# nmndeep/Robust-Segmentation

Hardware: AMD Instinct MI355X
Metric: SEA attack-iterations/sec (UperNet-CNX-T, 512x512) (higher is better)
Workload: dtype f32 (frozen-weight GEMMs on the 16-bit matrix cores by operand splitting: fp16x2 (22 significant bits per operand, 3 MFMA products) forward, fp16x2 (22 significant bits per operand, 3 MFMA products) input gradient; fp32 storage and accumulate)

## Files before the change

include/sea_hip.h:

```cpp
#ifndef SEA_HIP_H
#define SEA_HIP_H

#include <stddef.h>
#include <stdint.h>

#ifdef __cplusplus
extern "C" {
#endif

#define SEA_MODE_MASK_CE 0
#define SEA_MODE_MASK_CE_BAL 1
#define SEA_MODE_JS 2
#define SEA_MODE_CE 3

#define SEA_DTYPE_F32 0
#define SEA_DTYPE_BF16 1
#define SEA_DTYPE_F16 2

#define SEA_LAYOUT_NCHW 0
#define SEA_LAYOUT_NHWC 1

int sea_abi_version(void);
const char* sea_build_info(void);
#define SEA_CONFIG_XCD_ORDER 0
// ... 26 lines not shown
#define SEA_K2_VARIANT_DEFAULT 0u
#define SEA_K2_VEC_MASK 0xfu
#define SEA_K2_TUNE_SHIFT 4
#define SEA_K2_STREAM_SHIFT 8
#define SEA_K2_NO_SPLIT (15u << SEA_K2_STREAM_SHIFT)
#define SEA_K2_REG_ONLY 0x1000u
int sea_loss_fwd_bwd_tuned(const void* logits, int dtype, int layout, const void* y, int y_bytes,
                           const float* w, int mode, int track_mode, int B, int C, int64_t HW,
                           float grad_scale, void* dlogits, void* pred, int pred_bytes, float* loss_px,
                           void* workspace, size_t workspace_bytes, float* loss_sum, float* track_sum,
                           int32_t* n_correct, void* stream, int variant);
int sea_loss_plan(int dtype, int layout, int C, int64_t HW, int want_grad, size_t logits_addr, size_t dlogits_addr,
                  unsigned variant, int32_t out[8]);

size_t sea_loss_upsampled_workspace_bytes(int B, int C, int h, int w, int H, int W, int pow2);
int sea_loss_fwd_bwd_upsampled(const float* low, const void* y, int y_bytes, const float* w, int mode,
                               int track_mode, int B, int C, int h, int wl, int H, int W, float grad_scale,
                               float* dlow, void* pred, int pred_bytes, void* workspace,
                               size_t workspace_bytes, float* loss_sum, float* track_sum,
                               int32_t* n_correct, int pow2, void* stream);

int sea_class_counts(const void* pred, int pred_bytes, const void* y, int y_bytes, int B, int C,
                     int64_t HW, int mask_pred, int per_image, int64_t* inter, int64_t* pred_cnt,
                     int64_t* tgt_cnt, void* stream);
int sea_confusion(const void* pred, int pred_bytes, const void* y, int y_bytes, int64_t n, int C,
                  int64_t* hist, void* stream);

int sea_apgd_track(const float* loss_sum, const float* track_sum, const int32_t* n_correct,
                   const int32_t* n_ignored, int B, int64_t HW, int iter, int n_iter, int check_k,
                   int early_stop, int init, int32_t* acc_cnt, float* acc, float* loss_best,
                   float* loss_best_last, float* reduced_last, float* step, float* loss_steps,
                   uint8_t* flags, int32_t* done, const void* loss_workspace, void* stream);
int sea_apgd_linf_step_graph(const float* x, float* x_adv, float* x_old, const float* grad, const float* step_b,
                             const float* eps_dev, const int32_t* iter_dev, int B, int64_t n_per_img, void* stream);
int sea_apgd_track_graph(const float* loss_sum, const float* track_sum, const int32_t* n_correct,
                         const int32_t* n_ignored, int B, int64_t HW, int32_t* iter_dev, const int32_t* check_table,
                         const int32_t* n_iter_dev, int early_stop, int32_t* acc_cnt, float* acc, float* loss_best,
                         float* loss_best_last, float* reduced_last, float* step, float* loss_steps, uint8_t* flags,
                         int32_t* done, const void* loss_workspace, void* stream);
int sea_select_copy(const uint8_t* flags, float* x_adv, float* grad, float* x_best,
                    float* grad_best, float* x_best_adv, const void* pred, void* pred_best,
                    int pred_bytes, int B, int64_t n_per_img, int64_t HW, void* stream);

int sea_count_ignored(const void* y, int y_bytes, int B, int64_t HW, int32_t* n_ignored,
                      void* stream);

int sea_worst_miou_greedy(const float* ints, const float* unions, int A, int N, int C,
                          uint32_t* mt_state, int n_rounds, double* miou, int32_t* selected,
                          int32_t* rounds_run);

int sea_dwconv7x7(const float* x, const float* w, const float* bias, float* y, int B, int C, int H,
                  int W, int flip, void* stream);
int sea_dwconv7x7_nhwc(const float* x, const float* wt, const float* bias, float* y, int B, int C,
                       int H, int W, int flip, unsigned ab, void* stream);
int sea_dwconv7x7_nhwc_add(const float* x, const float* wt, const float* bias, const float* addend, float* y, int B,
                           int C, int H, int W, int flip, unsigned ab, void* stream);

int sea_upsample_bilinear_fwd(const float* x, float* y, int64_t planes, int h, int w, int H, int W,
                              void* stream);
int sea_upsample_bilinear_bwd(const float* gy, float* gx, int64_t planes, int h, int w, int H, int W,
                              void* stream);
int sea_upsample_bilinear_nhwc_fwd(const float* x, const float* residual, float* y, int B, int C, int h,
                                   int w, int H, int W, int64_t y_pixel_stride, void* stream);
int sea_upsample_bilinear_nhwc_bwd(const float* gy, float* gx, int B, int C, int h, int w, int H, int W,
                                   int64_t gy_pixel_stride, void* stream);
#define SEA_UP_NCHW_FWD 0
#define SEA_UP_NCHW_BWD 1
#define SEA_UP_NHWC_FWD 2
#define SEA_UP_NHWC_BWD 3
#define SEA_UP_TAP_FWD 4
#define SEA_UP_TAP_BWD 5
int sea_upsample_plan(int op, int64_t planes_or_batch, int C, int h, int w, int H, int W, int64_t pixel_stride,
                      size_t src_addr, size_t dst_addr, int general_only, int xcd_order, int32_t out[20]);

int64_t sea_wino_tiles(int B, int H, int W, int m);
int sea_wino_input_transform(const float* x, int64_t x_pixel_stride, const float* gate, const float* scale,
                             float* V, int64_t v_tile_stride, int B, int C, int H, int W, int m, int vec4, void* stream);
int sea_wino_filter_transform(const float* w, float* U, int Cout, int Cin, int m, int flip, void* stream);
int sea_wino_input_transform_amax(const float* x, int64_t x_pixel_stride, const float* gate, const float* scale, float* V,
                                  int64_t v_tile_stride, int B, int C, int H, int W, int m, int vec4, uint32_t* amax_out,
                                  void* stream);
int sea_wino_output_transform(const float* M, const float* addend, const float* scale, const float* bias,
                              int relu, float* y, int B, int C, int H, int W, int m, int vec4, void* stream);

int sea_layernorm_fwd(const float* x, const float* w, const float* b, float* y, float* mean, float* rstd,
                      int64_t rows, int C, float eps, void* stream);
int sea_layernorm_bwd(const float* g, const float* x, const float* w, const float* mean, const float* rstd,
                      float* dx, int64_t rows, int C, void* stream);

int64_t sea_layernorm_bwd_params_workspace(int64_t rows, int C);
int sea_layernorm_bwd_params(const float* g, const float* x, const float* w, const float* mean, const float* rstd,
                             float* dx, float* dw, float* db, float* ws, int64_t rows, int C, void* stream);

int sea_block_tail_fwd(const float* x, const float* y, const float* gamma, const float* s, float* out, int64_t rows, int HW,
                       int C, void* stream);
int64_t sea_block_tail_bwd_workspace(int64_t rows, int C);
int sea_block_tail_bwd(const float* g, const float* y, const float* gamma, const float* s, float* gy, float* ggamma, float* ws,
                       int64_t rows, int HW, int C, void* stream);

int64_t sea_dwconv7x7_nhwc_wgrad_workspace(int B, int C, int H);
int sea_dwconv7x7_nhwc_wgrad(const float* x, const float* gy, float* gw, float* gb, float* ws, int B, int C, int H, int W,
                             void* stream);

int sea_adaptive_avg_pool_nhwc_fwd(const float* x, float* out, int B, int C, int H, int W, int oh, int ow, void* stream);
int sea_adaptive_avg_pool_nhwc_bwd(const float* g, float* dx, int B, int C, int H, int W, int oh, int ow, void* stream);

int sea_stem_conv1_ln_gelu(const float* x, const float* w, const float* bias, const float* gamma, const float* beta,
                           float* y, float* a, int B, int CO, int H, int W, float eps, void* stream);
int sea_stem_conv1_bwd(const float* dy, const float* w, float* dx, int B, int CO, int H, int W, void* stream);
int sea_ln_gelu_cl_fwd(const float* y, const float* gamma, const float* beta, float* a, int a_nchw, int B, int C, int64_t HW,
                       float eps, void* stream);
int sea_ln_gelu_cl_bwd(const float* da, int a_nchw, const float* y, const float* gamma, const float* beta, float* dy, int B,
                       int C, int64_t HW, float eps, void* stream);

int sea_tap_gather_fwd(const float* G, float* extra, int accumulate, int B, int C, int h, int w, int H, int W,
                       int inner, void* stream);
int sea_tap_gather_bwd(const float* gz, float* dG, int B, int C, int h, int w, int H, int W, void* stream);
int sea_gate_scale(const float* g, const float* gate, const float* scale, float* out, int64_t pixels, int C,
                   void* stream);

int sea_nchw_to_nhwc(const float* in, const float* scale, float* out, int B, int C, int64_t HW, void* stream);
int sea_nhwc_to_nchw(const float* in, const float* scale, const float* residual, float* out, int B, int C,
                     int64_t HW, void* stream);

int sea_patch2x2(const float* src, float* dst, int B, int H, int W, int C, int inverse, void* stream);

int sea_attention_bwd_terms(const float* q, const float* k, const float* v, int64_t sb, int64_t sh, int64_t st, int B, int H,
                            int T, int D, float scale, const float* out, const float* grad_out, const float* lse,
                            float* delta, float* dq, float* dk, float* dv, int64_t gsb, int64_t gsh, int64_t gst,
                            int terms, void* stream);
int sea_attention_fwd_terms(const float* q, const float* k, const float* v, int64_t sb, int64_t sh, int64_t st, int B, int H,
                            int T, int D, float scale, float* out, float* lse, int terms, void* stream);
int sea_attention_fwd_f16(const float* q, const float* k, const float* v, int64_t sb, int64_t sh, int64_t st, int B, int H,
                          int T, int D, float scale, uint32_t* amax_ws, float* out, float* lse, void* stream);
int sea_attention_bwd_f16(const float* q, const float* k, const float* v, int64_t sb, int64_t sh, int64_t st, int B, int H,
                          int T, int D, float scale, const float* out, const float* grad_out, const float* lse,
                          float* delta, uint32_t* amax_ws, float* dq, float* dk, float* dv, int64_t gsb, int64_t gsh,
                          int64_t gst, void* stream);

#define SEA_GEMM_VARIANT_DEFAULT 0u
#define SEA_GEMM_PIPE_SINGLE 1u
#define SEA_GEMM_PIPE_PINGPONG 2u
#define SEA_GEMM_PIPE_BIG 3u
#define SEA_GEMM_PIPE_MASK 3u
#define SEA_GEMM_SHAPE16 4u
int sea_gemm_plan(int M, int N, int K, int terms, int batch, int64_t lda, int64_t ldc, int64_t ld_addend, int prologue, int fused,
                  unsigned variant, int32_t out[16]);
int64_t sea_gemm_split_packed_bytes(int N, int K, int terms);
int sea_absmax_bits(const float* A, int64_t lda, int M, int K, int batch, int64_t strideA, int rows_per_word,
                    uint32_t* out_bits, void* stream);
int sea_gemm_split_f16(const float* A, int64_t lda, const void* Wp, float* C, int64_t ldc, const float* bias, int relu, int M,
                       int N, int K, int batch, int64_t strideA, int64_t strideW_bytes, int64_t strideC,
                       const uint32_t* amax_bits, int amax_rows, uint32_t* out_amax, unsigned variant, void* stream);
int sea_gemm_split_pack(const float* W, int64_t ldw, int trans, int N, int K, int terms, void* out, void* stream);
int sea_gemm_splitk_reduce(const float* partial, int splits, int M, int N, const float* bias, const float* addend,
                           int64_t ld_addend, int relu, float* C, int64_t ldc, uint32_t* out_amax, void* stream);
typedef struct SeaGemmEpilogue {
  const float* addend;
  int64_t ld_addend, stride_addend;
  float* gelu_out;
  const float* gelu_grad_of;
  const float* a_gelu_grad_of;
  int a_gate;
  int a_gelu;
  float a_amax_mul;
  const float* a_amax_mul_dev;
} SeaGemmEpilogue;
int sea_gemm_split_fused(const float* A, int64_t lda, const void* Wp, float* C, int64_t ldc, const float* bias, int relu, int M,
                         int N, int K, int terms, int batch, int64_t strideA, int64_t strideW_bytes, int64_t strideC,
                         const uint32_t* amax_bits, int amax_rows, uint32_t* out_amax, const SeaGemmEpilogue* epi,
                         unsigned variant, void* stream);
int sea_gemm_split(const float* A, int64_t lda, const void* Wp, float* C, int64_t ldc, const float* bias, int relu, int M,
                   int N, int K, int terms, int batch, int64_t strideA, int64_t strideW_bytes, int64_t strideC,
                   unsigned variant, void* stream);
int sea_classifier_supported(int P, int K, int cls);
int sea_classifier_fwd(const float* y, const float* W, const float* bias, float* out, int B, int P, int K, int cls, void* stream);
int sea_classifier_bwd(const float* g, const float* W, float* gy, int B, int P, int K, int cls, const float* gate,
                       const float* gate_scale, void* stream);
int sea_mlp_fused_supported(int C, int H);
int sea_ln_mlp_fused_fwd(const float* x, int64_t ldx, const float* ln_w, const float* ln_b, float ln_eps, const void* W1p,
                         const float* b1, const void* W2p, const float* b2, const float* res, int64_t ldres, float* y,
                         int64_t ldy, int M, int C, int H, const uint32_t* amax_x, const uint32_t* amax_h, void* stream);
int sea_ln_mlp_fused_bwd(const float* g, int64_t ldg, const float* x, int64_t ldx, const float* ln_w, const float* ln_b,
                         float ln_eps, const void* W1p, const float* b1, const void* W2tp, const void* W1tp, float* dx,
                         int64_t lddx, int M, int C, int H, const uint32_t* amax_x, const float* amax_mul_dev, void* stream);
int sea_probe_gelu_mismatches(unsigned long long* out, void* stream);
int sea_probe_ln_rows(const float* x, const float* ln_w, const float* ln_b, float eps, int M, int C, float* yn, float* mean,
                      float* rstd, void* stream);
int sea_mlp_fused_stamps(int bwd, const float* g, int64_t ldg, const float* x, int64_t ldx, const void* W1p, const float* b1,
                         const void* W2p, const void* W1tp, const float* b2, const float* res, float* y, int M, int C,
                         const uint32_t* amax_x, const uint32_t* amax_h, const float* amax_mul_dev, unsigned long long* dbg,
                         void* stream);
int sea_mlp_fused_fwd(const float* x, int64_t ldx, const void* W1p, const float* b1, const void* W2p, const float* b2,
                      const float* res, int64_t ldres, float* y, int64_t ldy, int M, int C, int H, const uint32_t* amax_x,
                      const uint32_t* amax_h, void* stream);
int sea_mlp_fused_bwd(const float* g, int64_t ldg, const float* x, int64_t ldx, const void* W1p, const float* b1,
                      const void* W2tp, const void* W1tp, float* dx, int64_t lddx, int M, int C, int H,
                      const uint32_t* amax_x, const float* amax_mul_dev, void* stream);
int sea_probe_stream_copy(const void* src, void* dst, size_t bytes, int non_temporal, void* stream);
int sea_probe_stream_read(const void* src, float* sink, size_t bytes, void* stream);

#define SEA_MSF_MAX_CLASSES 192
int sea_msf_resize_input(const float* x, float* y, float* y_flip, int64_t planes, int h, int w, int H, int W,
                         void* stream);
int sea_msf_accumulate(const float* logits, float* score, int B, int C, int hl, int wl, int Hs, int Ws, int H, int W,
                       int flip, void* stream);

#define SEA_SW_MAX_ANCHORS 32
int sea_sw_merge(const float* logits, float* out, int B, int C, int hl, int wl, int ws, const int* h_anchors, int n_h,
                 const int* w_anchors, int n_w, int H, int W, int flip, int softmax, int accumulate, void* stream);
int sea_sw_finish(const float* avg, float* score, int B, int C, int H, int W, int Ho, int Wo, int flip, int accumulate,
                  void* stream);

int sea_psp_polyphase_split(const float* x, float* y, int B, int H, int W, int C, int d, int first_only, void* stream);
int sea_psp_polyphase_merge(const float* y, float* x, int B, int H, int W, int C, int d, int first_only, void* stream);
int sea_psp_upsample_ac(const float* x, float* y, int64_t planes, int h, int w, int H, int W, void* stream);
int sea_psp_upsample_ac_bwd(const float* gy, float* gx, float* work, int64_t planes, int h, int w, int H, int W,
                            void* stream);
int sea_psp_upsample_ac_nhwc(const float* x, float* y, int B, int C, int h, int w, int H, int W, int S, void* stream);
int sea_psp_upsample_ac_nhwc_bwd(const float* gy, float* gx, float* work, int B, int C, int h, int w, int H, int W,
                                 int S, void* stream);
int sea_psp_add_relu(const float* a, const float* r, float* y, int64_t n, void* stream);
int sea_psp_add_relu_bwd(const float* gy, const float* y, float* gx, int64_t n, void* stream);

int64_t sea_bn_train_workspace_floats(int64_t M, int C);
int sea_bn_train_fwd(const float* x, const float* r, const float* gamma, const float* beta, float* y, float* mean,
                     float* invstd, float* scale, float* running_mean, float* running_var, int64_t* num_batches_tracked,
                     float* work, int64_t M, int C, float eps, float momentum, int relu, void* stream);
int sea_bn_train_bwd(const float* g, const float* x, const float* y, const float* mean, const float* invstd,
                     const float* scale, float* dx, float* dgamma, float* dbeta, float* gr, float* work, int64_t M, int C,
                     int relu, void* stream);

size_t sea_train_ce_workspace_bytes(int B, int64_t HW);
int sea_train_ce_fwd(const void* logits, int dtype, const int64_t* y, const float* w, int64_t ignore_label, float thresh,
                     int reduce_mean, int B, int C, int64_t HW, float* loss_px, void* workspace, size_t workspace_bytes,
                     void* words, void* stream);
int sea_train_ohem_select(float* loss_px, int64_t N, void* workspace, size_t workspace_bytes, void* words, void* stream);
int sea_train_ce_bwd(const void* logits, int dtype, const int64_t* y, const float* w, int64_t ignore_label, int ohem,
                     int B, int C, int64_t HW, const float* loss_px, const float* g, const void* words, void* dlogits,
                     void* stream);

int sea_train_ce_up_tile(int C, int h, int w, int H, int W);
size_t sea_train_ce_up_workspace_bytes(int B, int C, int h, int w, int H, int W);
int sea_train_ce_up_fwd(const float* low, const int64_t* y, const float* wgt, int64_t ignore_label, float thresh,
                        int reduce_mean, int B, int C, int h, int w, int H, int W, float* loss_px, void* workspace,
                        size_t workspace_bytes, void* words, void* stream);
int sea_train_ce_up_bwd(const float* low, const int64_t* y, const float* wgt, int64_t ignore_label, int ohem, int B, int C,
                        int h, int w, int H, int W, const float* loss_px, const float* g, const void* words, float* dlow,
                        void* workspace, size_t workspace_bytes, void* stream);

int sea_train_ce_up_ac_tile(int C, int h, int w, int H, int W);
size_t sea_train_ce_up_ac_workspace_bytes(int B, int C, int h, int w, int H, int W);
int sea_train_ce_up_ac_fwd(const float* low, const int64_t* y, const float* wgt, int64_t ignore_label, float thresh,
                           int reduce_mean, int B, int C, int h, int w, int H, int W, float* loss_px, void* workspace,
                           size_t workspace_bytes, void* words, void* stream);
int sea_train_ce_up_ac_bwd(const float* low, const int64_t* y, const float* wgt, int64_t ignore_label, int ohem, int B,
                           int C, int h, int w, int H, int W, const float* loss_px, const float* g, const void* words,
                           float* dlow, void* workspace, size_t workspace_bytes, void* stream);

int sea_train_ce_up_pow2_supported(int C, int h, int w, int H, int W);
size_t sea_train_ce_up_pow2_workspace_bytes(int B, int C, int h, int w, int H, int W);
// ... 10 lines not shown
```

robust-segmentation_amd/csrc/classifier.hip:

```cpp
#include "sea_common.h"

namespace sea {

typedef float cf32x16 __attribute__((ext_vector_type(16)));
typedef float cf32x4 __attribute__((ext_vector_type(4)));

constexpr int CLS_MAX = 32;

__global__ __launch_bounds__(256, 2) void classifier_fwd_kernel(const float* __restrict__ y, const float* __restrict__ W,
                                                                const float* __restrict__ bias, float* __restrict__ out,
                                                                int tiles, int P, int K, int cls) {
  extern __shared__ __attribute__((aligned(16))) char cls_smem[];
  const int ldw = K + 4;
  float* const Ws = (float*)cls_smem;
  for (int i = threadIdx.x; i < CLS_MAX * (K / 4); i += 256) {
    const int c = i / (K / 4), k4 = i - c * (K / 4);
    const cf32x4 v = c < cls ? *(const cf32x4*)(W + (int64_t)c * K + 4 * k4) : cf32x4{0.f, 0.f, 0.f, 0.f};
    *(cf32x4*)(Ws + c * ldw + 4 * k4) = v;
  }
  __syncthreads();
  const int lane = threadIdx.x & 63, wave = threadIdx.x >> 6;
  const int r = lane & 31, h = lane >> 5;
  const float* const wrow = Ws + r * ldw + 4 * h;
  const int tiles_per_img = P / 32;
  for (int t = blockIdx.x * 4 + wave; t < tiles; t += gridDim.x * 4) {
    const float* const yrow = y + ((int64_t)t * 32 + r) * K + 4 * h;
    cf32x16 acc;
#pragma unroll
    for (int e = 0; e < 16; ++e) acc[e] = 0.f;
    cf32x4 cur[8], nxt[8];
#pragma unroll
    for (int i = 0; i < 8; ++i) cur[i] = *(const cf32x4*)(yrow + 8 * i);
    for (int kk = 0; kk < K; kk += 64) {
      if (kk + 64 < K) {
#pragma unroll
        for (int i = 0; i < 8; ++i) nxt[i] = *(const cf32x4*)(yrow + kk + 64 + 8 * i);
      }
#pragma unroll
      for (int i = 0; i < 8; ++i) {
        const cf32x4 a = *(const cf32x4*)(wrow + kk + 8 * i);
#pragma unroll
        for (int e = 0; e < 4; ++e) acc = __builtin_amdgcn_mfma_f32_32x32x2f32(a[e], cur[i][e], acc, 0, 0, 0);
      }
#pragma unroll
      for (int i = 0; i < 8; ++i) cur[i] = nxt[i];
    }
    const int b = t / tiles_per_img, p0 = (t - b * tiles_per_img) * 32;
    float* const ob = out + (int64_t)b * cls * P + p0 + r;
#pragma unroll
    for (int e = 0; e < 16; ++e) {
      const int c = (e & 3) + 8 * (e >> 2) + 4 * h;
      if (c < cls) ob[(int64_t)c * P] = acc[e] + (bias ? bias[c] : 0.f);
    }
  }
}

template <bool GATE>
__global__ __launch_bounds__(256, 2) void classifier_bwd_kernel(const float* __restrict__ g, const float* __restrict__ W,
                                                                float* __restrict__ gy, int tiles, int P, int K, int cls,
                                                                const float* __restrict__ gate, const float* __restrict__ scale) {
  extern __shared__ __attribute__((aligned(16))) char cls_smem[];
  const int ldw = K + 32;
  const int pairs = (cls + 1) / 2;
  float* const Ws = (float*)cls_smem;
  for (int i = threadIdx.x; i < 2 * pairs * (K / 4); i += 256) {
    const int c = i / (K / 4), k4 = i - c * (K / 4);
    const cf32x4 v = c < cls ? *(const cf32x4*)(W + (int64_t)c * K + 4 * k4) : cf32x4{0.f, 0.f, 0.f, 0.f};
    *(cf32x4*)(Ws + c * ldw + 4 * k4) = v;
  }
  __syncthreads();
  const int lane = threadIdx.x & 63, wave = threadIdx.x >> 6;
  const int r = lane & 31, h = lane >> 5;
  const int tiles_per_img = P / 32;
  for (int t = blockIdx.x * 4 + wave; t < tiles; t += gridDim.x * 4) {
    const int b = t / tiles_per_img, p0 = (t - b * tiles_per_img) * 32;
    const float* const gb = g + (int64_t)b * cls * P + p0 + r;
    float a[CLS_MAX / 2];
#pragma unroll
    for (int s = 0; s < CLS_MAX / 2; ++s) {
      const int c = 2 * s + h;
      a[s] = (s < pairs && c < cls) ? gb[(int64_t)c * P] : 0.f;
    }
    float* const orow = gy + ((int64_t)t * 32 + 4 * h) * K + r;
    const float* const grow = GATE ? gate + ((int64_t)t * 32 + 4 * h) * K + r : nullptr;
    for (int n0 = 0; n0 < K; n0 += 128) {
      cf32x16 acc[4];
      float gt[GATE ? 4 : 1][GATE ? 16 : 1];
      float sc[4];
#pragma unroll
      for (int nt = 0; nt < 4; ++nt) {
#pragma unroll
        for (int e = 0; e < 16; ++e) acc[nt][e] = 0.f;
        if constexpr (GATE) {
          if (n0 + 32 * nt < K) {
            sc[nt] = scale[n0 + 32 * nt + r];
#pragma unroll
            for (int e = 0; e < 16; ++e) gt[nt][e] = grow[(int64_t)((e & 3) + 8 * (e >> 2)) * K + n0 + 32 * nt];
          }
        }
      }
#pragma unroll
      for (int s = 0; s < CLS_MAX / 2; ++s) {
        if (s < pairs) {
          const float* const wr = Ws + (2 * s + h) * ldw + n0 + r;
#pragma unroll
          for (int nt = 0; nt < 4; ++nt)
            if (n0 + 32 * nt < K) acc[nt] = __builtin_amdgcn_mfma_f32_32x32x2f32(a[s], wr[32 * nt], acc[nt], 0, 0, 0);
        }
      }
#pragma unroll
      for (int nt = 0; nt < 4; ++nt) {
        if (n0 + 32 * nt < K) {
#pragma unroll
          for (int e = 0; e < 16; ++e) {
            const int64_t o = (int64_t)((e & 3) + 8 * (e >> 2)) * K + n0 + 32 * nt;
            if constexpr (GATE)
              orow[o] = gt[nt][e] > 0.f ? acc[nt][e] * sc[nt] : 0.f;
            else
              orow[o] = acc[nt][e];
          }
        }
      }
    }
  }
}

}

using namespace sea;

extern "C" int sea_classifier_supported(int P, int K, int cls) {
  return (P > 0 && (P % 32) == 0 && K >= 64 && (K % 64) == 0 && K <= 1024 && cls >= 1 && cls <= CLS_MAX) ? 1 : 0;
}

static int classifier_grid(int tiles) {
  const int blocks = (tiles + 3) / 4;
  return blocks < 512 ? blocks : 512;
}

extern "C" int sea_classifier_fwd(const float* y, const float* W, const float* bias, float* out, int B, int P, int K, int cls,
                                  void* stream) {
  SEA_CHECK_ARG(y && W && out && B > 0 && sea_classifier_supported(P, K, cls));
  SEA_CHECK_ARG(((((uintptr_t)y) | ((uintptr_t)W)) & 15) == 0 && (int64_t)B * P / 32 < (1ll << 30));
  const int tiles = (int)((int64_t)B * P / 32);
  const int lds = CLS_MAX * (K + 4) * 4;
  static bool attr_set_dev[64] = {};
  int dev = 0;
  (void)hipGetDevice(&dev);
  if (!attr_set_dev[dev & 63]) {
    (void)hipFuncSetAttribute((const void*)classifier_fwd_kernel, hipFuncAttributeMaxDynamicSharedMemorySize, CLS_MAX * (1024 + 4) * 4);
    attr_set_dev[dev & 63] = true;
  }
  hipLaunchKernelGGL(classifier_fwd_kernel, dim3(classifier_grid(tiles)), dim3(256), (size_t)lds, (hipStream_t)stream, y, W, bias, out,
                     tiles, P, K, cls);
  SEA_RETURN_LAST();
}

extern "C" int sea_classifier_bwd(const float* g, const float* W, float* gy, int B, int P, int K, int cls, const float* gate,
                                  const float* gate_scale, void* stream) {
  SEA_CHECK_ARG(g && W && gy && B > 0 && sea_classifier_supported(P, K, cls) && ((gate == nullptr) == (gate_scale == nullptr)));
  SEA_CHECK_ARG((((uintptr_t)W) & 15) == 0 && (int64_t)B * P / 32 < (1ll << 30));
  const int tiles = (int)((int64_t)B * P / 32);
  const int lds = 2 * ((cls + 1) / 2) * (K + 32) * 4;
  static bool attr_set_dev[64] = {};
  int dev = 0;
  (void)hipGetDevice(&dev);
  if (!attr_set_dev[dev & 63]) {
    (void)hipFuncSetAttribute((const void*)classifier_bwd_kernel<false>, hipFuncAttributeMaxDynamicSharedMemorySize, CLS_MAX * (1024 + 32) * 4);
    (void)hipFuncSetAttribute((const void*)classifier_bwd_kernel<true>, hipFuncAttributeMaxDynamicSharedMemorySize, CLS_MAX * (1024 + 32) * 4);
    attr_set_dev[dev & 63] = true;
  }
  if (gate)
    hipLaunchKernelGGL(classifier_bwd_kernel<true>, dim3(classifier_grid(tiles)), dim3(256), (size_t)lds, (hipStream_t)stream, g, W, gy,
                       tiles, P, K, cls, gate, gate_scale);
  else
    hipLaunchKernelGGL(classifier_bwd_kernel<false>, dim3(classifier_grid(tiles)), dim3(256), (size_t)lds, (hipStream_t)stream, g, W, gy,
                       tiles, P, K, cls, gate, gate_scale);
  SEA_RETURN_LAST();
}
```

robust-segmentation_amd/csrc/fpn_fused.hip:

```cpp
#include "sea_common.h"
#include <utility>
#include "bilinear_map.h"
#include "upsample_plan.h"

namespace sea {

constexpr int kTB = kTapBlock;

typedef float tg_f4 __attribute__((ext_vector_type(4)));

template <int N, typename F, int... I>
__device__ __forceinline__ void tg_static_for_impl(F&& f, std::integer_sequence<int, I...>) {
  (f(std::integral_constant<int, I>{}), ...);
}
template <int N, typename F>
__device__ __forceinline__ void tg_static_for(F&& f) {
  tg_static_for_impl<N>(f, std::make_integer_sequence<int, N>{});
}

template <int S>
struct TgAxis {
  static constexpr int LOG = Pow2<S>::LOG;
  static constexpr int base(int u0) { return (u0 >> LOG) - 1; }
  static constexpr int k(int u0, int q) { return ((u0 + q) >> LOG) - (u0 >> LOG); }
// ... 200 lines not shown
__global__ __launch_bounds__(256) void tap_gather_bwd_pow2_kernel(const float4* __restrict__ gz, float4* __restrict__ dG,
                                                                  int CG, int h, int w, int64_t total, int xcd,
                                                                  Divs3 dv) {
  constexpr int T = 2 * S, TW = T + 2;
  const int H = h * S, W = w * S;
  const IndexRange rg = xcd_range(total, xcd);
  const bool fast = total < kFastIndexLimit;
  for (int64_t i = rg.begin; i < rg.end; i += rg.stride) {
    const Index4 ix = split_index(i, dv, fast);
    const int cg = ix.c0, xq = ix.c1, yq = ix.c2;
    const int b = (int)ix.c3;
    const bool eL = xq == 0, eR = xq == w - 1, eT = yq == 0, eB = yq == h - 1;
    const int Q0 = S * xq - S / 2 - 1, R0 = S * yq - S / 2 - 1;
    float wxe[T];
#pragma unroll
    for (int t = 0; t < T; ++t) wxe[t] = pow2_tap_weight<S>(t, eL, eR);
    const float4* gb = gz + ((int64_t)b * H * W + Q0) * CG + cg;
    float4 acc[3][3];
#pragma unroll
    for (int a = 0; a < 3; ++a)
#pragma unroll
      for (int bq = 0; bq < 3; ++bq) acc[a][bq] = make_float4(0.f, 0.f, 0.f, 0.f);
#pragma unroll 1
    for (int u = 0; u < TW; ++u) {
      const int R = R0 + u;
      if (R < 0 || R >= H) continue;
      const float wy0 = pow2_tap_weight<S>(u - 2, eT, eB), wy1 = pow2_tap_weight<S>(u - 1, eT, eB),
                  wy2 = pow2_tap_weight<S>(u, eT, eB);
      const float4* row = gb + (int64_t)R * W * CG;
      float4 g[TW];
#pragma unroll
      for (int v = 0; v < TW; ++v) {
        const int Q = Q0 + v;
        g[v] = make_float4(0.f, 0.f, 0.f, 0.f);
        if (Q >= 0 && Q < W) g[v] = row[(int64_t)v * CG];
      }
      float4 rb[3];
#pragma unroll
      for (int bq = 0; bq < 3; ++bq) {
        rb[bq] = make_float4(0.f, 0.f, 0.f, 0.f);
#pragma unroll
        for (int t = 0; t < T; ++t) {
          const int v = t + 2 - bq;
          rb[bq].x = fmaf(wxe[t], g[v].x, rb[bq].x);
          rb[bq].y = fmaf(wxe[t], g[v].y, rb[bq].y);
          rb[bq].z = fmaf(wxe[t], g[v].z, rb[bq].z);
          rb[bq].w = fmaf(wxe[t], g[v].w, rb[bq].w);
        }
      }
#pragma unroll
      for (int bq = 0; bq < 3; ++bq) {
        acc[0][bq].x = fmaf(wy0, rb[bq].x, acc[0][bq].x);
        acc[0][bq].y = fmaf(wy0, rb[bq].y, acc[0][bq].y);
        acc[0][bq].z = fmaf(wy0, rb[bq].z, acc[0][bq].z);
        acc[0][bq].w = fmaf(wy0, rb[bq].w, acc[0][bq].w);
        acc[1][bq].x = fmaf(wy1, rb[bq].x, acc[1][bq].x);
        acc[1][bq].y = fmaf(wy1, rb[bq].y, acc[1][bq].y);
        acc[1][bq].z = fmaf(wy1, rb[bq].z, acc[1][bq].z);
        acc[1][bq].w = fmaf(wy1, rb[bq].w, acc[1][bq].w);
        acc[2][bq].x = fmaf(wy2, rb[bq].x, acc[2][bq].x);
        acc[2][bq].y = fmaf(wy2, rb[bq].y, acc[2][bq].y);
        acc[2][bq].z = fmaf(wy2, rb[bq].z, acc[2][bq].z);
        acc[2][bq].w = fmaf(wy2, rb[bq].w, acc[2][bq].w);
      }
    }
    float4* out = dG + (((int64_t)b * h + yq) * w + xq) * 9 * CG + cg;
#pragma unroll
    for (int a = 0; a < 3; ++a)
#pragma unroll
      for (int bq = 0; bq < 3; ++bq) out[(a * 3 + bq) * CG] = acc[a][bq];
  }
}

__global__ __launch_bounds__(256) void gate_scale_kernel(const float4* __restrict__ g, const float4* __restrict__ gate,
                                                         const float4* __restrict__ scale, float4* __restrict__ out, int CG,
                                                         int64_t total) {
  for (int64_t i = (int64_t)blockIdx.x * blockDim.x + threadIdx.x; i < total; i += (int64_t)gridDim.x * blockDim.x) {
    const float4 s = scale[i % CG], gv = g[i], t = gate[i];
    out[i] = make_float4(t.x > 0.f ? gv.x * s.x : 0.f, t.y > 0.f ? gv.y * s.y : 0.f, t.z > 0.f ? gv.z * s.z : 0.f,
                         t.w > 0.f ? gv.w * s.w : 0.f);
  }
}

}

using namespace sea;

extern "C" int sea_tap_gather_fwd(const float* G, float* extra, int accumulate, int B, int C, int h, int w, int H, int W,
                                  int inner, void* stream) {
  SEA_CHECK_ARG(G && extra);
  UpsamplePlan pl;
  SEA_CHECK_ARG(upsample_plan(UpsampleQuery{SEA_UP_TAP_FWD, B, C, h, w, H, W, 0, (uintptr_t)G, (uintptr_t)extra,
                                            process_config().upsample_general != 0, process_config().xcd_order}, &pl) == 0);
  dispatch_s<0, 4, 8>(pl.S, [&](auto S) {
    launch_planned(tap_gather_fwd_kernel<decltype(S)::value>, pl, 1, stream, (const float4*)G, (float4*)extra, accumulate, C / 4,
                   h, w, H, W, (float)h / (float)H, (float)w / (float)W, pl.nbh, pl.nbw, pl.total, pl.xo,
                   divs3(C / 4, pl.nbw, pl.nbh), inner ? 1 : 0);
  });
  SEA_RETURN_LAST();
}

extern "C" int sea_tap_gather_bwd(const float* gz, float* dG, int B, int C, int h, int w, int H, int W, void* stream) {
  SEA_CHECK_ARG(gz && dG);
  UpsamplePlan pl;
  SEA_CHECK_ARG(upsample_plan(UpsampleQuery{SEA_UP_TAP_BWD, B, C, h, w, H, W, 0, (uintptr_t)gz, (uintptr_t)dG,
                                            process_config().upsample_general != 0, process_config().xcd_order}, &pl) == 0);
  if (pl.kernel == UPK_TAP_BWD_POW2)
    dispatch_s<4, 8>(pl.S, [&](auto S) {
      launch_planned(tap_gather_bwd_pow2_kernel<decltype(S)::value>, pl, 1, stream, (const float4*)gz, (float4*)dG, C / 4, h, w,
                     pl.total, pl.xo, divs3(C / 4, w, h));
    });
  else
    launch_planned(tap_gather_bwd_kernel, pl, 1, stream, (const float4*)gz, (float4*)dG, C / 4, h, w, H, W, (float)h / (float)H,
                   (float)w / (float)W, pl.total, pl.xo, divs3(C / 4, w, h));
  SEA_RETURN_LAST();
}

extern "C" int sea_gate_scale(const float* g, const float* gate, const float* scale, float* out, int64_t pixels, int C,
                              void* stream) {
  SEA_CHECK_ARG(g && gate && scale && out && pixels > 0 && C > 0 && (C % 4) == 0);
  SEA_CHECK_ARG(((((uintptr_t)g) | ((uintptr_t)gate) | ((uintptr_t)scale) | ((uintptr_t)out)) & 15) == 0);
  const int64_t total = pixels * (C / 4);
  hipLaunchKernelGGL(gate_scale_kernel, dim3(grid_for(total, 256 * 2)), dim3(256), 0, (hipStream_t)stream,
                     (const float4*)g, (const float4*)gate, (const float4*)scale, (float4*)out, C / 4, total);
  SEA_RETURN_LAST();
}
```

robust-segmentation_amd/csrc/wino_kernels.hip:

```cpp
#include "sea_common.h"

namespace sea {

__host__ __device__ constexpr float wino_bt(int m, int i, int k) {
  if (m == 2) {
    constexpr float T[4][4] = {{1, 0, -1, 0}, {0, 1, 1, 0}, {0, -1, 1, 0}, {0, 1, 0, -1}};
    return T[i][k];
  }
  constexpr float T[6][6] = {{4, 0, -5, 0, 1, 0},  {0, -4, -4, 1, 1, 0}, {0, 4, -4, -1, 1, 0},
                             {0, -2, -1, 2, 1, 0}, {0, 2, -1, -2, 1, 0}, {0, 4, 0, -5, 0, 1}};
  return T[i][k];
}
__host__ __device__ constexpr float wino_g(int m, int i, int k) {
  if (m == 2) {
    constexpr float T[4][3] = {{1, 0, 0}, {0.5f, 0.5f, 0.5f}, {0.5f, -0.5f, 0.5f}, {0, 0, 1}};
    return T[i][k];
  }
  constexpr float T[6][3] = {{1.f / 4, 0, 0},           {-1.f / 6, -1.f / 6, -1.f / 6}, {-1.f / 6, 1.f / 6, -1.f / 6},
                             {1.f / 24, 1.f / 12, 1.f / 6}, {1.f / 24, -1.f / 12, 1.f / 6},  {0, 0, 1}};
  return T[i][k];
}
__host__ __device__ constexpr float wino_at(int m, int i, int k) {
  if (m == 2) {
    constexpr float T[2][4] = {{1, 1, 1, 0}, {0, 1, -1, -1}};
    return T[i][k];
  }
  constexpr float T[4][6] = {{1, 1, 1, 1, 1, 0}, {0, 1, -1, 2, -2, 0}, {0, 1, 1, 4, 4, 0}, {0, 1, -1, 8, -8, 1}};
  return T[i][k];
}

template <int VEC>
__device__ __forceinline__ void axpy(float c, const float (&v)[VEC], float (&acc)[VEC], bool& first) {
  if (c == 0.f) return;
#pragma unroll
  for (int e = 0; e < VEC; ++e) acc[e] = first ? c * v[e] : fmaf(c, v[e], acc[e]);
  first = false;
}

template <int VEC>
struct VecT;
template <>
struct VecT<4> {
  using type = float4;
};
template <>
struct VecT<2> {
  using type = float2;
};

template <int VEC>
__device__ __forceinline__ void vload(const float* p, float (&v)[VEC]) {
  const typename VecT<VEC>::type r = *(const typename VecT<VEC>::type*)p;
  const float* rp = (const float*)&r;
#pragma unroll
  for (int e = 0; e < VEC; ++e) v[e] = rp[e];
}
template <int VEC>
__device__ __forceinline__ void vstore(float* p, const float (&v)[VEC]) {
  typename VecT<VEC>::type r;
  float* rp = (float*)&r;
#pragma unroll
  for (int e = 0; e < VEC; ++e) rp[e] = v[e];
  *(typename VecT<VEC>::type*)p = r;
}

template <int M, int VEC>
__global__ __launch_bounds__(256) void wino_input_kernel(const float* __restrict__ x, const float* __restrict__ gate,
                                                         const float* __restrict__ scale, float* __restrict__ V, int C,
                                                         int H, int W, int nTh, int nTw, int64_t T, int64_t total,
                                                         int64_t xps, int64_t vts, int xcd, Divs3 dv,
                                                         uint32_t* __restrict__ amax_out) {
  constexpr int A = M + 2;
  const bool fast = total < kFastIndexLimit;
  const IndexRange rg = xcd_range(total, xcd);
  for (int64_t idx = rg.begin; idx < rg.end; idx += rg.stride) {
    const Index4 ix = split_index(idx, dv, fast);
    const int cg = ix.c0, tx = ix.c1, ty = ix.c2;
    const int b = (int)ix.c3;
    const int64_t t = ((int64_t)b * nTh + ty) * nTw + tx;
    const int y0 = ty * M - 1, x0 = tx * M - 1;
    const int64_t base = (int64_t)b * H * W * C + (int64_t)cg * VEC;
    const float* xb = x + (int64_t)b * H * W * xps + (int64_t)cg * VEC;
    float sc[VEC];
#pragma unroll
    for (int e = 0; e < VEC; ++e) sc[e] = scale ? scale[cg * VEC + e] : 1.f;
    float d[A][A][VEC];
#pragma unroll
    for (int i = 0; i < A; ++i) {
      const int yy = y0 + i;
#pragma unroll
      for (int j = 0; j < A; ++j) {
        const int xx = x0 + j;
        if (yy >= 0 && yy < H && xx >= 0 && xx < W) {
          vload<VEC>(xb + ((int64_t)yy * W + xx) * xps, d[i][j]);
          if (gate) {
            float gt[VEC];
            vload<VEC>(gate + base + ((int64_t)yy * W + xx) * C, gt);
#pragma unroll
            for (int e = 0; e < VEC; ++e) d[i][j][e] = gt[e] > 0.f ? d[i][j][e] * sc[e] : 0.f;
          }
        } else {
#pragma unroll
          for (int e = 0; e < VEC; ++e) d[i][j][e] = 0.f;
        }
      }
    }
    float tmp[A][A][VEC];
#pragma unroll
    for (int i = 0; i < A; ++i)
#pragma unroll
      for (int j = 0; j < A; ++j) {
        bool first = true;
#pragma unroll
        for (int k = 0; k < A; ++k) axpy<VEC>(wino_bt(M, i, k), d[k][j], tmp[i][j], first);
      }
    float* vb = V + t * vts + (int64_t)cg * VEC;
    uint32_t vmax = 0;
#pragma unroll
    for (int i = 0; i < A; ++i)
#pragma unroll
      for (int j = 0; j < A; ++j) {
        float v[VEC];
        bool first = true;
#pragma unroll
        for (int k = 0; k < A; ++k) axpy<VEC>(wino_bt(M, j, k), tmp[i][k], v, first);
        vstore<VEC>(vb + (int64_t)(i * A + j) * T * vts, v);
#pragma unroll
        for (int e = 0; e < VEC; ++e) {
          const uint32_t b = __float_as_uint(v[e]) & 0x7fffffffu;
          vmax = b > vmax ? b : vmax;
        }
      }
    if (amax_out != nullptr) {
      const int ti = (int)t;
      const bool whole = __ballot(1) == ~0ull && __all(ti == __shfl(ti, 0, 64));
      if (whole) {
#pragma unroll
        for (int o = 32; o > 0; o >>= 1) {
          const uint32_t other = (uint32_t)__shfl_xor((int)vmax, o, 64);
          vmax = other > vmax ? other : vmax;
        }
        if ((threadIdx.x & 63) == 0) atomicMax(amax_out + t, vmax);
      } else {
        atomicMax(amax_out + t, vmax);
      }
    }
  }
}

template <int M, int VEC>
__global__ __launch_bounds__(256) void wino_input_cols_kernel(const float* __restrict__ x, const float* __restrict__ gate,
                                                              const float* __restrict__ scale, float* __restrict__ V, int C,
                                                              int H, int W, int nTh, int nTw, int64_t T, int64_t total,
                                                              int64_t xps, int64_t vts, int xcd, Divs3 dv,
                                                              uint32_t* __restrict__ amax_out) {
  constexpr int A = M + 2;
  const bool fast = total < kFastIndexLimit;
  const IndexRange rg = xcd_range(total, xcd);
  for (int64_t idx = rg.begin; idx < rg.end; idx += rg.stride) {
    const Index4 ix = split_index(idx, dv, fast);
    const int cg = ix.c0, tx = ix.c1, ty = ix.c2;
    const int b = (int)ix.c3;
    const int64_t t = ((int64_t)b * nTh + ty) * nTw + tx;
    const int y0 = ty * M - 1, x0 = tx * M - 1;
    const int64_t base = (int64_t)b * H * W * C + (int64_t)cg * VEC;
    const float* xb = x + (int64_t)b * H * W * xps + (int64_t)cg * VEC;
    float sc[VEC];
#pragma unroll
    for (int e = 0; e < VEC; ++e) sc[e] = scale ? scale[cg * VEC + e] : 1.f;
    float tmp[A][A][VEC];
#pragma unroll
    for (int j = 0; j < A; ++j) {
      const int xx = x0 + j;
      float col[A][VEC];
#pragma unroll
      for (int i = 0; i < A; ++i) {
        const int yy = y0 + i;
        if (yy >= 0 && yy < H && xx >= 0 && xx < W) {
          vload<VEC>(xb + ((int64_t)yy * W + xx) * xps, col[i]);
          if (gate) {
            float gt[VEC];
            vload<VEC>(gate + base + ((int64_t)yy * W + xx) * C, gt);
#pragma unroll
            for (int e = 0; e < VEC; ++e) col[i][e] = gt[e] > 0.f ? col[i][e] * sc[e] : 0.f;
          }
        } else {
#pragma unroll
          for (int e = 0; e < VEC; ++e) col[i][e] = 0.f;
        }
      }
#pragma unroll
      for (int i = 0; i < A; ++i) {
        bool first = true;
#pragma unroll
        for (int k = 0; k < A; ++k) axpy<VEC>(wino_bt(M, i, k), col[k], tmp[i][j], first);
      }
    }
    float* vb = V + t * vts + (int64_t)cg * VEC;
    uint32_t vmax = 0;
#pragma unroll
    for (int i = 0; i < A; ++i)
#pragma unroll
      for (int j = 0; j < A; ++j) {
        float v[VEC];
        bool first = true;
#pragma unroll
        for (int k = 0; k < A; ++k) axpy<VEC>(wino_bt(M, j, k), tmp[i][k], v, first);
        vstore<VEC>(vb + (int64_t)(i * A + j) * T * vts, v);
#pragma unroll
        for (int e = 0; e < VEC; ++e) {
          const uint32_t b = __float_as_uint(v[e]) & 0x7fffffffu;
          vmax = b > vmax ? b : vmax;
        }
      }
    if (amax_out != nullptr) {
      const int ti = (int)t;
      const bool whole = __ballot(1) == ~0ull && __all(ti == __shfl(ti, 0, 64));
      if (whole) {
#pragma unroll
        for (int o = 32; o > 0; o >>= 1) {
          const uint32_t other = (uint32_t)__shfl_xor((int)vmax, o, 64);
          vmax = other > vmax ? other : vmax;
        }
        if ((threadIdx.x & 63) == 0) atomicMax(amax_out + t, vmax);
      } else {
        atomicMax(amax_out + t, vmax);
      }
    }
  }
}

template <int M, int VEC>
__global__ __launch_bounds__(256) void wino_output_kernel(const float* __restrict__ Mx, const float* __restrict__ addend,
                                                          const float* __restrict__ scale,
                                                          const float* __restrict__ bias, int relu,
                                                          float* __restrict__ y, int C, int H, int W, int nTh, int nTw,
                                                          int64_t T, int64_t total, Divs3 dv) {
  constexpr int A = M + 2;
  const bool fast = total < kFastIndexLimit;
  for (int64_t idx = (int64_t)blockIdx.x * blockDim.x + threadIdx.x; idx < total;
       idx += (int64_t)gridDim.x * blockDim.x) {
    const Index4 ix = split_index(idx, dv, fast);
    const int cg = ix.c0, tx = ix.c1, ty = ix.c2;
    const int b = (int)ix.c3;
    const int64_t t = ((int64_t)b * nTh + ty) * nTw + tx;
    const float* mb = Mx + t * C + (int64_t)cg * VEC;
    float tmp[M][A][VEC];
#pragma unroll
    for (int j = 0; j < A; ++j) {
      float col[A][VEC];
#pragma unroll
      for (int i = 0; i < A; ++i) vload<VEC>(mb + (int64_t)(i * A + j) * T * C, col[i]);
#pragma unroll
      for (int p = 0; p < M; ++p) {
        bool first = true;
#pragma unroll
        for (int i = 0; i < A; ++i) axpy<VEC>(wino_at(M, p, i), col[i], tmp[p][j], first);
      }
    }
    float bv[VEC], sv[VEC];
#pragma unroll
    for (int e = 0; e < VEC; ++e) {
      bv[e] = bias ? bias[cg * VEC + e] : 0.f;
      sv[e] = scale ? scale[cg * VEC + e] : 1.f;
    }
    float* yb = y + (int64_t)b * H * W * C + (int64_t)cg * VEC;
#pragma unroll
    for (int p = 0; p < M; ++p) {
      const int yy = ty * M + p;
#pragma unroll
      for (int q = 0; q < M; ++q) {
        const int xx = tx * M + q;
        float o[VEC];
        bool first = true;
#pragma unroll
        for (int j = 0; j < A; ++j) axpy<VEC>(wino_at(M, q, j), tmp[p][j], o, first);
        if (addend && yy < H && xx < W) {
          float ad[VEC];
          vload<VEC>(addend + (int64_t)b * H * W * C + ((int64_t)yy * W + xx) * C + (int64_t)cg * VEC, ad);
#pragma unroll
          for (int e = 0; e < VEC; ++e) o[e] += ad[e];
        }
#pragma unroll
        for (int e = 0; e < VEC; ++e) {
          o[e] = scale ? fmaf(o[e], sv[e], bv[e]) : o[e] + bv[e];
          if (relu) o[e] = fmaxf(o[e], 0.f);
        }
        if (yy < H && xx < W) vstore<VEC>(yb + ((int64_t)yy * W + xx) * C, o);
      }
    }
  }
}

template <int M>
__global__ __launch_bounds__(256) void wino_filter_kernel(const float* __restrict__ w, float* __restrict__ U, int Cout,
                                                          int Cin, int flip) {
  constexpr int A = M + 2;
  const int64_t n = (int64_t)Cout * Cin;
  for (int64_t idx = (int64_t)blockIdx.x * blockDim.x + threadIdx.x; idx < n; idx += (int64_t)gridDim.x * blockDim.x) {
    const int c = (int)(idx % Cin);
    const int o = (int)(idx / Cin);
    float g[3][3];
#pragma unroll
    for (int a = 0; a < 3; ++a)
#pragma unroll
      for (int bq = 0; bq < 3; ++bq) g[a][bq] = w[idx * 9 + (flip ? (2 - a) * 3 + (2 - bq) : a * 3 + bq)];
    float tmp[A][3];
#pragma unroll
    for (int i = 0; i < A; ++i)
#pragma unroll
      for (int j = 0; j < 3; ++j) {
        float s = 0.f;
#pragma unroll
        for (int k = 0; k < 3; ++k)
          if (wino_g(M, i, k) != 0.f) s = fmaf(wino_g(M, i, k), g[k][j], s);
        tmp[i][j] = s;
      }
    const int64_t off = flip ? (int64_t)o * Cin + c : (int64_t)c * Cout + o;
#pragma unroll
    for (int i = 0; i < A; ++i)
#pragma unroll
      for (int j = 0; j < A; ++j) {
        float s = 0.f;
#pragma unroll
        for (int k = 0; k < 3; ++k)
          if (wino_g(M, j, k) != 0.f) s = fmaf(wino_g(M, j, k), tmp[i][k], s);
        U[(int64_t)(i * A + j) * n + off] = s;
      }
  }
}

}

using namespace sea;

static bool wino_dims(int B, int C, int H, int W, int m, int vec, int* nTh, int* nTw, int64_t* T) {
  if (!(B > 0 && C > 0 && H > 0 && W > 0 && (m == 2 || m == 4) && (C % vec) == 0)) return false;
  *nTh = (H + m - 1) / m;
  *nTw = (W + m - 1) / m;
  *T = (int64_t)B * *nTh * *nTw;
  return true;
}

extern "C" int64_t sea_wino_tiles(int B, int H, int W, int m) {
  if (!(B > 0 && H > 0 && W > 0 && (m == 2 || m == 4))) return 0;
  return (int64_t)B * ((H + m - 1) / m) * ((W + m - 1) / m);
}

static int wino_input_impl(const float* x, int64_t x_pixel_stride, const float* gate, const float* scale, float* V,
                           int64_t v_tile_stride, int B, int C, int H, int W, int m, int vec4, uint32_t* amax_out, void* stream);

extern "C" int sea_wino_input_transform(const float* x, int64_t x_pixel_stride, const float* gate, const float* scale,
                                        float* V, int64_t v_tile_stride, int B, int C, int H, int W, int m, int vec4,
                                        void* stream) {
  return wino_input_impl(x, x_pixel_stride, gate, scale, V, v_tile_stride, B, C, H, W, m, vec4, nullptr, stream);
}

extern "C" int sea_wino_input_transform_amax(const float* x, int64_t x_pixel_stride, const float* gate, const float* scale,
                                             float* V, int64_t v_tile_stride, int B, int C, int H, int W, int m, int vec4,
                                             uint32_t* amax_out, void* stream) {
  SEA_CHECK_ARG(amax_out != nullptr);
  return wino_input_impl(x, x_pixel_stride, gate, scale, V, v_tile_stride, B, C, H, W, m, vec4, amax_out, stream);
}

static int wino_input_impl(const float* x, int64_t x_pixel_stride, const float* gate, const float* scale, float* V,
                           int64_t v_tile_stride, int B, int C, int H, int W, int m, int vec4, uint32_t* amax_out, void* stream) {
  int nTh, nTw;
  int64_t T;
  SEA_CHECK_ARG(x && V && wino_dims(B, C, H, W, m, 4, &nTh, &nTw, &T));
  SEA_CHECK_ARG(x_pixel_stride >= C && (x_pixel_stride % 4) == 0);
  SEA_CHECK_ARG(v_tile_stride >= C && (v_tile_stride % 4) == 0);
  SEA_CHECK_ARG(((((uintptr_t)x) | ((uintptr_t)V) | ((uintptr_t)gate)) & 15) == 0);
  if (m == 2) {
    const int64_t total = T * (C / 4);
    hipLaunchKernelGGL((wino_input_kernel<2, 4>), dim3(grid_for_xcd(total, 256)), dim3(256), 0, (hipStream_t)stream, x, gate,
                       scale, V, C, H, W, nTh, nTw, T, total, x_pixel_stride, v_tile_stride, xcd_order_enabled() == 2, divs3(C / 4, nTw, nTh),
                       amax_out);
  } else if (vec4) {
    const int64_t total = T * (C / 4);
    hipLaunchKernelGGL((wino_input_cols_kernel<4, 4>), dim3(grid_for_xcd(total, 256)), dim3(256), 0, (hipStream_t)stream, x, gate,
                       scale, V, C, H, W, nTh, nTw, T, total, x_pixel_stride, v_tile_stride, xcd_order_enabled() == 2, divs3(C / 4, nTw, nTh),
                       amax_out);
  } else {
    const int64_t total = T * (C / 2);
    hipLaunchKernelGGL((wino_input_kernel<4, 2>), dim3(grid_for_xcd(total, 256)), dim3(256), 0, (hipStream_t)stream, x, gate,
                       scale, V, C, H, W, nTh, nTw, T, total, x_pixel_stride, v_tile_stride, xcd_order_enabled() == 2, divs3(C / 2, nTw, nTh),
                       amax_out);
  }
  SEA_RETURN_LAST();
}

extern "C" int sea_wino_output_transform(const float* Mx, const float* addend, const float* scale, const float* bias,
                                         int relu, float* y, int B, int C, int H, int W, int m, int vec4, void* stream) {
  int nTh, nTw;
  int64_t T;
  SEA_CHECK_ARG(Mx && y && wino_dims(B, C, H, W, m, 4, &nTh, &nTw, &T));
  SEA_CHECK_ARG(((((uintptr_t)Mx) | ((uintptr_t)y) | ((uintptr_t)addend)) & 15) == 0);
  if (m == 2) {
    const int64_t total = T * (C / 4);
    hipLaunchKernelGGL((wino_output_kernel<2, 4>), dim3(grid_for(total, 256)), dim3(256), 0, (hipStream_t)stream, Mx,
                       addend, scale, bias, relu, y, C, H, W, nTh, nTw, T, total, divs3(C / 4, nTw, nTh));
  } else if (vec4) {
    const int64_t total = T * (C / 4);
    hipLaunchKernelGGL((wino_output_kernel<4, 4>), dim3(grid_for(total, 256)), dim3(256), 0, (hipStream_t)stream, Mx,
                       addend, scale, bias, relu, y, C, H, W, nTh, nTw, T, total, divs3(C / 4, nTw, nTh));
  } else {
    const int64_t total = T * (C / 2);
    hipLaunchKernelGGL((wino_output_kernel<4, 2>), dim3(grid_for(total, 256)), dim3(256), 0, (hipStream_t)stream, Mx,
                       addend, scale, bias, relu, y, C, H, W, nTh, nTw, T, total, divs3(C / 2, nTw, nTh));
  }
  SEA_RETURN_LAST();
}

extern "C" int sea_wino_filter_transform(const float* w, float* U, int Cout, int Cin, int m, int flip, void* stream) {
  SEA_CHECK_ARG(w && U && Cout > 0 && Cin > 0 && (m == 2 || m == 4));
  const int64_t n = (int64_t)Cout * Cin;
  if (m == 2)
    hipLaunchKernelGGL((wino_filter_kernel<2>), dim3(grid_for(n, 256)), dim3(256), 0, (hipStream_t)stream, w, U, Cout,
                       Cin, flip);
  else
    hipLaunchKernelGGL((wino_filter_kernel<4>), dim3(grid_for(n, 256)), dim3(256), 0, (hipStream_t)stream, w, U, Cout,
                       Cin, flip);
  SEA_RETURN_LAST();
}
```

robust-segmentation_amd/semseg/_native.py:

```python
from __future__ import annotations

import ctypes as C
import os
from typing import Optional

import torch

_PKG = os.path.dirname(os.path.dirname(os.path.abspath(__file__)))
LIB_PATH = os.environ.get("SEA_HIP_LIB", os.path.join(_PKG, "lib", "libsea_hip.so"))

MODE_BY_NAME = {"mask-ce-avg": 0, "mask-ce-bal": 1, "js-avg": 2, "ce": 3, "ce-avg": 3}
DTYPE_CODE = {torch.float32: 0, torch.bfloat16: 1, torch.float16: 2}
LAYOUT_NCHW, LAYOUT_NHWC = 0, 1

_lib = None

_vp, _i, _i64, _f, _sz, _u = C.c_void_p, C.c_int, C.c_int64, C.c_float, C.c_size_t, C.c_uint
_SIGS = {
    "sea_abi_version": (C.c_int, []),
    "sea_build_info": (C.c_char_p, []),
    "sea_fastdiv_magic": (_i, [C.c_uint32, C.POINTER(C.c_uint32), C.POINTER(C.c_uint32)]),
    "sea_apgd_linf_step": (_i, [_vp, _vp, _vp, _vp, _vp, _f, _f, _vp, _i, _i64, _vp]),
    "sea_apgd_l2_workspace_bytes": (_i64, [_i]),
    "sea_apgd_l2_step": (_i, [_vp, _vp, _vp, _vp, _vp, _f, _f, _vp, _vp, _i, _i64, _vp]),
    "sea_linf_random_start": (_i, [_vp, _vp, _f, _vp, _i64, _vp]),
    "sea_linf_project": (_i, [_vp, _vp, _f, _vp, _i64, _vp]),
    "sea_pgd_linf_step": (_i, [_vp, _vp, _vp, _f, _f, _vp, _vp, _i, _i64, _vp]),
    "sea_loss_workspace_bytes": (_sz, [_i, _i64]),
    "sea_loss_fwd_bwd": (_i, [_vp, _i, _i, _vp, _i, _vp, _i, _i, _i, _i, _i64, _f, _vp, _vp, _i, _vp, _vp, _sz,
                              _vp, _vp, _vp, _vp]),
    "sea_loss_fwd_bwd_tuned": (_i, [_vp, _i, _i, _vp, _i, _vp, _i, _i, _i, _i, _i64, _f, _vp, _vp, _i, _vp, _vp,
                                    _sz, _vp, _vp, _vp, _vp, _i]),
    "sea_loss_plan": (_i, [_i, _i, _i, _i64, _i, _sz, _sz, _u, C.POINTER(C.c_int32)]),
    "sea_loss_upsampled_workspace_bytes": (_sz, [_i, _i, _i, _i, _i, _i, _i]),
    "sea_loss_fwd_bwd_upsampled": (_i, [_vp, _vp, _i, _vp, _i, _i, _i, _i, _i, _i, _i, _i, _f, _vp, _vp, _i, _vp, _sz, _vp,
                                        _vp, _vp, _i, _vp]),
    "sea_class_counts": (_i, [_vp, _i, _vp, _i, _i, _i, _i64, _i, _i, _vp, _vp, _vp, _vp]),
    "sea_confusion": (_i, [_vp, _i, _vp, _i, _i64, _i, _vp, _vp]),
    "sea_apgd_track": (_i, [_vp, _vp, _vp, _vp, _i, _i64, _i, _i, _i, _i, _i, _vp, _vp, _vp, _vp, _vp, _vp, _vp,
                            _vp, _vp, _vp, _vp]),
    "sea_apgd_linf_step_graph": (_i, [_vp, _vp, _vp, _vp, _vp, _vp, _vp, _i, _i64, _vp]),
    "sea_apgd_track_graph": (_i, [_vp, _vp, _vp, _vp, _i, _i64, _vp, _vp, _vp, _i, _vp, _vp, _vp, _vp, _vp, _vp, _vp, _vp,
                                  _vp, _vp, _vp]),
    "sea_select_copy": (_i, [_vp, _vp, _vp, _vp, _vp, _vp, _vp, _vp, _i, _i, _i64, _i64, _vp]),
    "sea_count_ignored": (_i, [_vp, _i, _i, _i64, _vp, _vp]),
    "sea_worst_miou_greedy": (_i, [_vp, _vp, _i, _i, _i, _vp, _i, _vp, _vp, _vp]),
    "sea_dwconv7x7": (_i, [_vp, _vp, _vp, _vp, _i, _i, _i, _i, _i, _vp]),
    "sea_dwconv7x7_nhwc": (_i, [_vp, _vp, _vp, _vp, _i, _i, _i, _i, _i, _u, _vp]),
    "sea_dwconv7x7_nhwc_add": (_i, [_vp, _vp, _vp, _vp, _vp, _i, _i, _i, _i, _i, _u, _vp]),
    "sea_nchw_to_nhwc": (_i, [_vp, _vp, _vp, _i, _i, _i64, _vp]),
    "sea_nhwc_to_nchw": (_i, [_vp, _vp, _vp, _vp, _i, _i, _i64, _vp]),
    "sea_upsample_bilinear_fwd": (_i, [_vp, _vp, _i64, _i, _i, _i, _i, _vp]),
    "sea_upsample_bilinear_bwd": (_i, [_vp, _vp, _i64, _i, _i, _i, _i, _vp]),
    "sea_layernorm_fwd": (_i, [_vp, _vp, _vp, _vp, _vp, _vp, _i64, _i, _f, _vp]),
    "sea_layernorm_bwd": (_i, [_vp, _vp, _vp, _vp, _vp, _vp, _i64, _i, _vp]),
    "sea_layernorm_bwd_params_workspace": (_i64, [_i64, _i]),
    "sea_layernorm_bwd_params": (_i, [_vp, _vp, _vp, _vp, _vp, _vp, _vp, _vp, _vp, _i64, _i, _vp]),
    "sea_block_tail_fwd": (_i, [_vp, _vp, _vp, _vp, _vp, _i64, _i, _i, _vp]),
    "sea_block_tail_bwd_workspace": (_i64, [_i64, _i]),
    "sea_block_tail_bwd": (_i, [_vp, _vp, _vp, _vp, _vp, _vp, _vp, _i64, _i, _i, _vp]),
    "sea_dwconv7x7_nhwc_wgrad_workspace": (_i64, [_i, _i, _i]),
    "sea_dwconv7x7_nhwc_wgrad": (_i, [_vp, _vp, _vp, _vp, _vp, _i, _i, _i, _i, _vp]),
    "sea_adaptive_avg_pool_nhwc_fwd": (_i, [_vp, _vp, _i, _i, _i, _i, _i, _i, _vp]),
    "sea_adaptive_avg_pool_nhwc_bwd": (_i, [_vp, _vp, _i, _i, _i, _i, _i, _i, _vp]),
    "sea_stem_conv1_ln_gelu": (_i, [_vp, _vp, _vp, _vp, _vp, _vp, _vp, _i, _i, _i, _i, _f, _vp]),
    "sea_stem_conv1_bwd": (_i, [_vp, _vp, _vp, _i, _i, _i, _i, _vp]),
    "sea_ln_gelu_cl_fwd": (_i, [_vp, _vp, _vp, _vp, _i, _i, _i, _i64, _f, _vp]),
    "sea_ln_gelu_cl_bwd": (_i, [_vp, _i, _vp, _vp, _vp, _vp, _i, _i, _i64, _f, _vp]),
    "sea_wino_tiles": (_i64, [_i, _i, _i, _i]),
    "sea_wino_input_transform": (_i, [_vp, _i64, _vp, _vp, _vp, _i64, _i, _i, _i, _i, _i, _i, _vp]),
    "sea_wino_filter_transform": (_i, [_vp, _vp, _i, _i, _i, _i, _vp]),
    "sea_wino_output_transform": (_i, [_vp, _vp, _vp, _vp, _i, _vp, _i, _i, _i, _i, _i, _i, _vp]),
    "sea_tap_gather_fwd": (_i, [_vp, _vp, _i, _i, _i, _i, _i, _i, _i, _i, _vp]),
    "sea_tap_gather_bwd": (_i, [_vp, _vp, _i, _i, _i, _i, _i, _i, _vp]),
    "sea_gate_scale": (_i, [_vp, _vp, _vp, _vp, _i64, _i, _vp]),
    "sea_upsample_bilinear_nhwc_fwd": (_i, [_vp, _vp, _vp, _i, _i, _i, _i, _i, _i, _i64, _vp]),
    "sea_upsample_bilinear_nhwc_bwd": (_i, [_vp, _vp, _i, _i, _i, _i, _i, _i, _i64, _vp]),
    "sea_upsample_plan": (_i, [_i, _i64, _i, _i, _i, _i, _i, _i64, _sz, _sz, _i, _i, C.POINTER(C.c_int32)]),
    "sea_patch2x2": (_i, [_vp, _vp, _i, _i, _i, _i, _i, _vp]),
    "sea_attention_bwd_terms": (_i, [_vp, _vp, _vp, _i64, _i64, _i64, _i, _i, _i, _i, _f, _vp, _vp, _vp, _vp, _vp, _vp, _vp,
                                     _i64, _i64, _i64, _i, _vp]),
    "sea_attention_fwd_terms": (_i, [_vp, _vp, _vp, _i64, _i64, _i64, _i, _i, _i, _i, _f, _vp, _vp, _i, _vp]),
    "sea_attention_fwd_f16": (_i, [_vp, _vp, _vp, _i64, _i64, _i64, _i, _i, _i, _i, _f, _vp, _vp, _vp, _vp]),
    "sea_attention_bwd_f16": (_i, [_vp, _vp, _vp, _i64, _i64, _i64, _i, _i, _i, _i, _f, _vp, _vp, _vp, _vp, _vp, _vp, _vp, _vp,
                                   _i64, _i64, _i64, _vp]),
    "sea_absmax_bits": (_i, [_vp, _i64, _i, _i, _i, _i64, _i, _vp, _vp]),
    "sea_gemm_split_f16": (_i, [_vp, _i64, _vp, _vp, _i64, _vp, _i, _i, _i, _i, _i, _i64, _i64, _i64, _vp, _i, _vp, _u, _vp]),
    "sea_wino_input_transform_amax": (_i, [_vp, _i64, _vp, _vp, _vp, _i64, _i, _i, _i, _i, _i, _i, _vp, _vp]),
    "sea_gemm_split_fused": (_i, [_vp, _i64, _vp, _vp, _i64, _vp, _i, _i, _i, _i, _i, _i, _i64, _i64, _i64, _vp, _i, _vp, _vp, _u, _vp]),
    "sea_gemm_splitk_reduce": (_i, [_vp, _i, _i, _i, _vp, _vp, _i64, _i, _vp, _i64, _vp, _vp]),
    "sea_gemm_split_packed_bytes": (_i64, [_i, _i, _i]),
    "sea_gemm_split_pack": (_i, [_vp, _i64, _i, _i, _i, _i, _vp, _vp]),
    "sea_gemm_split": (_i, [_vp, _i64, _vp, _vp, _i64, _vp, _i, _i, _i, _i, _i, _i, _i64, _i64, _i64, _u, _vp]),
    "sea_gemm_plan": (_i, [_i, _i, _i, _i, _i, _i64, _i64, _i64, _i, _i, _u, C.POINTER(C.c_int32)]),
    "sea_mlp_fused_supported": (_i, [_i, _i]),
    "sea_classifier_supported": (_i, [_i, _i, _i]),
    "sea_classifier_fwd": (_i, [_vp, _vp, _vp, _vp, _i, _i, _i, _i, _vp]),
    "sea_classifier_bwd": (_i, [_vp, _vp, _vp, _i, _i, _i, _i, _vp, _vp, _vp]),
    "sea_probe_gelu_mismatches": (_i, [_vp, _vp]),
    "sea_probe_ln_rows": (_i, [_vp, _vp, _vp, _f, _i, _i, _vp, _vp, _vp, _vp]),
    "sea_mlp_fused_stamps": (_i, [_i, _vp, _i64, _vp, _i64, _vp, _vp, _vp, _vp, _vp, _vp, _vp, _i, _i, _vp, _vp, _vp, _vp, _vp]),
    "sea_mlp_fused_fwd": (_i, [_vp, _i64, _vp, _vp, _vp, _vp, _vp, _i64, _vp, _i64, _i, _i, _i, _vp, _vp, _vp]),
    "sea_mlp_fused_bwd": (_i, [_vp, _i64, _vp, _i64, _vp, _vp, _vp, _vp, _vp, _i64, _i, _i, _i, _vp, _vp, _vp]),
    "sea_ln_mlp_fused_fwd": (_i, [_vp, _i64, _vp, _vp, _f, _vp, _vp, _vp, _vp, _vp, _i64, _vp, _i64, _i, _i, _i, _vp, _vp, _vp]),
    "sea_ln_mlp_fused_bwd": (_i, [_vp, _i64, _vp, _i64, _vp, _vp, _f, _vp, _vp, _vp, _vp, _vp, _i64, _i, _i, _i, _vp, _vp, _vp]),
    "sea_process_config": (_i, [_i]),
    "sea_probe_stream_copy": (_i, [_vp, _vp, _sz, _i, _vp]),
    "sea_probe_stream_read": (_i, [_vp, _vp, _sz, _vp]),
    "sea_msf_resize_input": (_i, [_vp, _vp, _vp, _i64, _i, _i, _i, _i, _vp]),
    "sea_msf_accumulate": (_i, [_vp, _vp, _i, _i, _i, _i, _i, _i, _i, _i, _i, _vp]),
    "sea_psp_polyphase_split": (_i, [_vp, _vp, _i, _i, _i, _i, _i, _i, _vp]),
    "sea_psp_polyphase_merge": (_i, [_vp, _vp, _i, _i, _i, _i, _i, _i, _vp]),
    "sea_psp_upsample_ac": (_i, [_vp, _vp, _i64, _i, _i, _i, _i, _vp]),
    "sea_psp_upsample_ac_bwd": (_i, [_vp, _vp, _vp, _i64, _i, _i, _i, _i, _vp]),
    "sea_psp_upsample_ac_nhwc": (_i, [_vp, _vp, _i, _i, _i, _i, _i, _i, _i, _vp]),
    "sea_psp_upsample_ac_nhwc_bwd": (_i, [_vp, _vp, _vp, _i, _i, _i, _i, _i, _i, _i, _vp]),
    "sea_psp_add_relu": (_i, [_vp, _vp, _vp, _i64, _vp]),
    "sea_psp_add_relu_bwd": (_i, [_vp, _vp, _vp, _i64, _vp]),
    "sea_bn_train_workspace_floats": (_i64, [_i64, _i]),
    "sea_bn_train_fwd": (_i, [_vp, _vp, _vp, _vp, _vp, _vp, _vp, _vp, _vp, _vp, _vp, _vp, _i64, _i, _f, _f, _i, _vp]),
    "sea_bn_train_bwd": (_i, [_vp, _vp, _vp, _vp, _vp, _vp, _vp, _vp, _vp, _vp, _vp, _i64, _i, _i, _vp]),
    "sea_train_ce_workspace_bytes": (_sz, [_i, _i64]),
    "sea_train_ce_fwd": (_i, [_vp, _i, _vp, _vp, _i64, _f, _i, _i, _i, _i64, _vp, _vp, _sz, _vp, _vp]),
    "sea_train_ohem_select": (_i, [_vp, _i64, _vp, _sz, _vp, _vp]),
    "sea_train_ce_bwd": (_i, [_vp, _i, _vp, _vp, _i64, _i, _i, _i, _i64, _vp, _vp, _vp, _vp, _vp]),
    "sea_train_ce_up_tile": (_i, [_i, _i, _i, _i, _i]),
    "sea_train_ce_up_workspace_bytes": (_sz, [_i, _i, _i, _i, _i, _i]),
    "sea_train_ce_up_fwd": (_i, [_vp, _vp, _vp, _i64, _f, _i, _i, _i, _i, _i, _i, _i, _vp, _vp, _sz, _vp, _vp]),
    "sea_train_ce_up_bwd": (_i, [_vp, _vp, _vp, _i64, _i, _i, _i, _i, _i, _i, _i, _vp, _vp, _vp, _vp, _vp, _sz, _vp]),
    "sea_train_ce_up_ac_tile": (_i, [_i, _i, _i, _i, _i]),
    "sea_train_ce_up_ac_workspace_bytes": (_sz, [_i, _i, _i, _i, _i, _i]),
    "sea_train_ce_up_ac_fwd": (_i, [_vp, _vp, _vp, _i64, _f, _i, _i, _i, _i, _i, _i, _i, _vp, _vp, _sz, _vp, _vp]),
    "sea_train_ce_up_ac_bwd": (_i, [_vp, _vp, _vp, _i64, _i, _i, _i, _i, _i, _i, _i, _vp, _vp, _vp, _vp, _vp, _sz, _vp]),
    "sea_train_ce_up_pow2_supported": (_i, [_i, _i, _i, _i, _i]),
    "sea_train_ce_up_pow2_workspace_bytes": (_sz, [_i, _i, _i, _i, _i, _i]),
    "sea_train_ce_up_pow2_fwd": (_i, [_vp, _vp, _vp, _i64, _i, _i, _i, _i, _i, _i, _vp, _vp, _sz, _vp, _vp]),
    "sea_train_ce_up_pow2_scale": (_i, [_vp, _vp, _vp, _vp, _i64, _vp]),
    "sea_sw_merge": (_i, [_vp, _vp, _i, _i, _i, _i, _i, C.POINTER(C.c_int), _i, C.POINTER(C.c_int), _i, _i, _i, _i, _i, _i,
                          _vp]),
    "sea_sw_finish": (_i, [_vp, _vp, _i, _i, _i, _i, _i, _i, _i, _i, _vp]),
}
EXPORTS = tuple(_SIGS)


class SeaNativeError(RuntimeError):
    pass


def lib():
    global _lib
    if _lib is None:
        if not os.path.exists(LIB_PATH):
            raise SeaNativeError(
                f"libsea_hip.so not found at {LIB_PATH}: build it with "
                "`python robust-segmentation_amd/build_native.py` (there is no CPU fallback)")
        h = C.CDLL(LIB_PATH)
        for name, (res, args) in _SIGS.items():
            fn = getattr(h, name)
            fn.restype, fn.argtypes = res, args
        _lib = h
    return _lib


def _check(rc: int, what: str):
    if rc != 0:
        raise SeaNativeError(f"{what} failed with hipError {rc}")


def _dev(*ts):
    cur = None
    for t in ts:
        if t is None:
            continue
        if not t.is_cuda:
            raise SeaNativeError("libsea_hip works on HIP device tensors only (no CPU fallback); got a CPU tensor")
        if cur is None:
            cur = torch.cuda.current_device()
        if t.device.index != cur:
            raise SeaNativeError(f"tensor on {t.device} but the current device is cuda:{cur}: call "
                                 "torch.cuda.set_device (or use `with torch.cuda.device(...)`) before the launch")

# ... 728 lines not shown

def upsample_bilinear_cl(x, size, out=None, residual=None):
    _dev(x, out, residual)
    if x.dtype != torch.float32 or cl_pixel_stride(x) != x.shape[1]:
        raise SeaNativeError("expected a dense channels_last float32 tensor with C % 4 == 0")
    B, Cc, h, w = x.shape
    H, W = int(size[0]), int(size[1])
    if out is None:
        out = torch.empty(B, Cc, H, W, dtype=torch.float32, device=x.device, memory_format=torch.channels_last)
    S = cl_pixel_stride(out)
    if tuple(out.shape) != (B, Cc, H, W) or S is None:
        raise SeaNativeError("out must be a (B,C,H,W) channels_last tensor or a channel slice of one")
    if residual is not None and (tuple(residual.shape) != (B, Cc, H, W) or cl_pixel_stride(residual) != Cc):
        raise SeaNativeError("residual must be a dense channels_last (B,C,H,W) float32 tensor")
    _check(lib().sea_upsample_bilinear_nhwc_fwd(_p(x), _p(residual), _p(out), B, Cc, h, w, H, W, S, _stream()),
           "sea_upsample_bilinear_nhwc_fwd")
    return out


def upsample_bilinear_backward_cl(gy, in_size):
    _dev(gy)
    S = cl_pixel_stride(gy)
    if S is None:
        raise SeaNativeError("expected a channels_last float32 tensor (or channel slice) with C % 4 == 0")
    B, Cc, H, W = gy.shape
    h, w = int(in_size[0]), int(in_size[1])
    gx = torch.empty(B, Cc, h, w, dtype=torch.float32, device=gy.device, memory_format=torch.channels_last)
    _check(lib().sea_upsample_bilinear_nhwc_bwd(_p(gy), _p(gx), B, Cc, h, w, H, W, S, _stream()),
           "sea_upsample_bilinear_nhwc_bwd")
    return gx


UPSAMPLE_OPS = ("nchw_fwd", "nchw_bwd", "nhwc_fwd", "nhwc_bwd", "tap_fwd", "tap_bwd")
UPSAMPLE_KERNELS = ("nchw_fwd_general", "nchw_fwd_pow2", "nchw_fwd_cells", "nchw_bwd_general", "nchw_bwd_rows", "nchw_bwd_pow2",
                    "nhwc_fwd", "nhwc_fwd_cells", "nhwc_bwd_general", "nhwc_bwd_small", "nhwc_bwd_pow2",
                    "tap_fwd", "tap_bwd_general", "tap_bwd_pow2")
_UPSAMPLE_PLAN_FIELDS = ("kernel", "S", "grid_x", "grid_y", "threads", "lds", "chunk", "nchunks", "total_lo", "total_hi", "xo", "nt",
                         "lcols", "RP", "bands", "per_xcd", "TI", "RMAX", "nbh", "nbw")


def upsample_plan(op: str, n: int, h: int, w: int, H: int, W: int, C_: int = 0, pixel_stride=None, src_addr: int = 0,
                  dst_addr: int = 0, general_only=None, xcd_order=None) -> dict:
    out = (C.c_int32 * len(_UPSAMPLE_PLAN_FIELDS))()
    L = lib()
    general_only = L.sea_process_config(1) if general_only is None else int(bool(general_only))
    xcd_order = L.sea_process_config(0) if xcd_order is None else int(xcd_order)
    rc = L.sea_upsample_plan(UPSAMPLE_OPS.index(op), n, C_, h, w, H, W, C_ if pixel_stride is None else pixel_stride, src_addr,
                             dst_addr, general_only, xcd_order, out)
    plan = dict(zip(_UPSAMPLE_PLAN_FIELDS, out), rc=rc)
    total = (plan.pop("total_hi") << 32) | (plan.pop("total_lo") & 0xffffffff)
    return dict(plan, kernel=UPSAMPLE_KERNELS[plan["kernel"]], total=total)


TAP_INNER = os.environ.get("SEA_TAP_INNER", "1")[:1] != "0"


def tap_gather(G, size, extra=None):
    _dev(G, extra)
    B, h, w, nine, Cc = G.shape
    H, W = int(size[0]), int(size[1])
    if nine != 9:
        raise SeaNativeError("tap_gather: G must be (B,h,w,9,C)")
    acc = extra is not None
    if extra is None:
        extra = torch.empty(B, Cc, H, W, dtype=torch.float32, device=G.device, memory_format=torch.channels_last)
    elif tuple(extra.shape) != (B, Cc, H, W) or cl_pixel_stride(extra) != Cc:
        raise SeaNativeError("tap_gather: extra must be a dense channels_last (B,C,H,W) float32 tensor")
    _check(lib().sea_tap_gather_fwd(_p(_f32c(G)), _p(extra), int(acc), B, Cc, h, w, H, W, int(TAP_INNER), _stream()),
           "sea_tap_gather_fwd")
    return extra


def tap_gather_backward(gz, coarse_size):
    _dev(gz)
    B, Cc, H, W = gz.shape
    if cl_pixel_stride(gz) != Cc:
        raise SeaNativeError("tap_gather_backward: dense channels_last float32 gradient expected")
    h, w = int(coarse_size[0]), int(coarse_size[1])
    dG = torch.empty(B, h, w, 9, Cc, dtype=torch.float32, device=gz.device)
    _check(lib().sea_tap_gather_bwd(_p(gz), _p(dG), B, Cc, h, w, H, W, _stream()), "sea_tap_gather_bwd")
    return dG


def gate_scale(g, gate, scale):
    _dev(g, gate, scale)
    B, Cc, H, W = g.shape
    if cl_pixel_stride(g) != Cc or cl_pixel_stride(gate) != Cc or gate.shape != g.shape or scale.numel() != Cc:
        raise SeaNativeError("gate_scale: dense channels_last float32 tensors of one shape expected")
    out = torch.empty_like(g)
    _check(lib().sea_gate_scale(_p(g), _p(gate), _p(_f32c(scale)), _p(out), B * H * W, Cc, _stream()), "sea_gate_scale")
    return out


def layernorm(x, weight, bias, eps: float):
    _dev(x, weight, bias)
    x = _f32c(x)
    Cc = x.shape[-1]
    rows = x.numel() // Cc
    y = torch.empty_like(x)
    mean = torch.empty(rows, dtype=torch.float32, device=x.device)
    rstd = torch.empty(rows, dtype=torch.float32, device=x.device)
    _check(lib().sea_layernorm_fwd(_p(x), _p(_f32c(weight)), _p(_f32c(bias)), _p(y), _p(mean), _p(rstd), rows, Cc,
                                   float(eps), _stream()), "sea_layernorm_fwd")
    return y, mean, rstd


def layernorm_backward(g, x, weight, mean, rstd):
    _dev(g, x, weight, mean, rstd)
    Cc = x.shape[-1]
    dx = torch.empty_like(x)
    _check(lib().sea_layernorm_bwd(_p(_f32c(g)), _p(_f32c(x)), _p(_f32c(weight)), _p(mean), _p(rstd), _p(dx),
                                   x.numel() // Cc, Cc, _stream()), "sea_layernorm_bwd")
    return dx


def layernorm_backward_params(g, x, weight, mean, rstd):
    _dev(g, x, weight, mean, rstd)
    Cc = x.shape[-1]
    rows = x.numel() // Cc
    L = lib()
    ws = torch.empty(int(L.sea_layernorm_bwd_params_workspace(rows, Cc)), dtype=torch.float32, device=x.device)
    dx = torch.empty_like(x)
    dw = torch.empty(Cc, dtype=torch.float32, device=x.device)
    db = torch.empty(Cc, dtype=torch.float32, device=x.device)
    _check(L.sea_layernorm_bwd_params(_p(_f32c(g)), _p(_f32c(x)), _p(_f32c(weight)), _p(mean), _p(rstd), _p(dx), _p(dw),
                                      _p(db), _p(ws), rows, Cc, _stream()), "sea_layernorm_bwd_params")
    return dx, dw, db


def _tail_args(x, y, gamma, s, what):
    if x.dim() != 4 or y.shape != x.shape or x.shape[-1] % 4 or x.shape[-1] > 1024 or x.numel() == 0:
        raise SeaNativeError(f"{what}: two (B,H,W,C) tensors of one shape, C % 4 == 0, C <= 1024")
    B, H, W, Cc = x.shape
    if gamma is not None and _f32c(gamma).shape != (Cc,):
        raise SeaNativeError(f"{what}: gamma must be (C)")
    if s is not None and _f32c(s).numel() != B:
        raise SeaNativeError(f"{what}: s must hold one factor per image")
    return B * H * W, H * W, Cc


def block_tail(x, y, gamma=None, s=None):
    _dev(x, y, gamma, s)
    rows, HW, Cc = _tail_args(x, y, gamma, s, "block_tail")
    out = torch.empty_like(x)
    _check(lib().sea_block_tail_fwd(_p(_f32c(x)), _p(_f32c(y)), _p(gamma), _p(s), _p(out), rows, HW, Cc, _stream()),
           "sea_block_tail_fwd")
    return out


def block_tail_backward(g, y, gamma=None, s=None, want_gamma: bool = False):
    _dev(g, y, gamma, s)
    rows, HW, Cc = _tail_args(g, g if y is None else y, gamma, s, "block_tail_backward")
    L = lib()
    gy = torch.empty_like(g)
    gg = ws = None
    if want_gamma:
        if y is None:
            raise SeaNativeError("block_tail_backward: the layer-scale gradient needs y")
        ws = torch.empty(int(L.sea_block_tail_bwd_workspace(rows, Cc)), dtype=torch.float32, device=g.device)
        gg = torch.empty(Cc, dtype=torch.float32, device=g.device)
    _check(L.sea_block_tail_bwd(_p(_f32c(g)), _p(None if y is None else _f32c(y)), _p(gamma), _p(s), _p(gy), _p(gg), _p(ws),
                                rows, HW, Cc, _stream()), "sea_block_tail_bwd")
    return gy, gg


def adaptive_avg_pool_nhwc(x, oh: int, ow: int):
    _dev(x)
    if x.dtype != torch.float32 or cl_pixel_stride(x) != x.shape[1]:
# ... 24 lines not shown
def _nhwc_dense(t):
    return t.dim() == 4 and t.is_contiguous(memory_format=torch.channels_last)


def _empty_cl(B, Cc, H, W, device):
    return torch.empty((B, H, W, Cc), dtype=torch.float32, device=device).permute(0, 3, 1, 2)


def stem_conv1_ln_gelu(x, weight, bias, gamma=None, beta=None, eps: float = 1e-6):
    _dev(x, weight, bias, gamma, beta)
    if x.dim() != 4 or x.shape[1] != 3 or tuple(weight.shape[1:]) != (3, 3, 3) or weight.shape[0] not in STEM_CONV1_CHANNELS:
        raise SeaNativeError("stem_conv1_ln_gelu: x (B,3,H,W) and weight (48,3,3,3) expected")
    x = _f32c(x)
    B, _, H, W = x.shape
    CO = weight.shape[0]
    y = _empty_cl(B, CO, (H - 1) // 2 + 1, (W - 1) // 2 + 1, x.device)
    a = torch.empty_like(y) if gamma is not None else None
    _check(lib().sea_stem_conv1_ln_gelu(_p(x), _p(_f32c(weight)), _p(_f32c(bias)) if bias is not None else None,
                                        _p(_f32c(gamma)) if gamma is not None else None,
                                        _p(_f32c(beta)) if gamma is not None else None, _p(y),
                                        _p(a) if a is not None else None, B, CO, H, W, float(eps), _stream()),
           "sea_stem_conv1_ln_gelu")
    return y, a


def stem_conv1_backward(dy, weight, H: int, W: int):
    _dev(dy, weight)
    B, CO, Ho, Wo = dy.shape
    if (Ho, Wo) != ((H - 1) // 2 + 1, (W - 1) // 2 + 1) or CO not in STEM_CONV1_CHANNELS:
        raise SeaNativeError("stem_conv1_backward: dy does not belong to an input of this size")
    if dy.dtype != torch.float32 or not _nhwc_dense(dy):
        raise SeaNativeError("stem_conv1_backward: dy must be float32 in channels_last memory")
    dx = torch.empty((B, 3, H, W), dtype=torch.float32, device=dy.device)
    _check(lib().sea_stem_conv1_bwd(_p(dy), _p(_f32c(weight)), _p(dx), B, CO, H, W, _stream()), "sea_stem_conv1_bwd")
    return dx


def ln_gelu_cl(y, gamma, beta, eps: float = 1e-6, out_nchw: bool = False):
    _dev(y, gamma, beta)
    if y.dtype != torch.float32 or not _nhwc_dense(y) or y.shape[1] not in LN_GELU_CL_CHANNELS:
        raise SeaNativeError("ln_gelu_cl: float32 (B,C,H,W) in channels_last memory with C in (48, 96) expected")
    B, Cc, H, W = y.shape
    a = torch.empty((B, Cc, H, W), dtype=torch.float32, device=y.device) if out_nchw else torch.empty_like(y)
    _check(lib().sea_ln_gelu_cl_fwd(_p(y), _p(_f32c(gamma)), _p(_f32c(beta)), _p(a), int(out_nchw), B, Cc, H * W, float(eps),
                                    _stream()), "sea_ln_gelu_cl_fwd")
    return a


def ln_gelu_cl_backward(da, y, gamma, beta, eps: float = 1e-6):
    _dev(da, y, gamma, beta)
    if da.dtype != torch.float32 or da.shape != y.shape or not _nhwc_dense(y):
        raise SeaNativeError("ln_gelu_cl_backward: da float32 of y's shape, y in channels_last memory")
    B, Cc, H, W = y.shape
    nchw = da.is_contiguous()
    if not nchw and not _nhwc_dense(da):
        raise SeaNativeError("ln_gelu_cl_backward: da must be NCHW-contiguous or channels_last")
    dy = torch.empty_like(y)
    _check(lib().sea_ln_gelu_cl_bwd(_p(da), int(nchw), _p(y), _p(_f32c(gamma)), _p(_f32c(beta)), _p(dy), B, Cc, H * W,
                                    float(eps), _stream()), "sea_ln_gelu_cl_bwd")
    return dy


def wino_filter(weight, m: int, flip: bool):
    _dev(weight)
    Cout, Cin, kh, kw = weight.shape
    if (kh, kw) != (3, 3):
        raise SeaNativeError("Winograd path is for 3x3 filters")
    A = m + 2
    U = torch.empty((A * A, Cout, Cin) if flip else (A * A, Cin, Cout), dtype=torch.float32, device=weight.device)
    _check(lib().sea_wino_filter_transform(_p(_f32c(weight)), _p(U), Cout, Cin, m, int(flip), _stream()),
           "sea_wino_filter_transform")
    return U


WINO_SPLIT_MIN_TILES = int(os.environ.get("SEA_WINO_SPLIT_MIN_TILES", "16"))
WINO_IN_VEC4 = int(os.environ.get("SEA_WINO_IN_VEC4", "1"))


def _wino_vector(v, n, what):
    if v is not None and (v.dtype != torch.float32 or v.numel() != n or not v.is_contiguous()):
        raise SeaNativeError(f"{what}: per-channel vectors must be contiguous float32 of the channel count")


def wino_input_transform(x, m: int, gate=None, gate_scale=None, vec4: int = None, amax=None, out=None):
    words = amax if isinstance(amax, torch.Tensor) else None
    _dev(x, gate, gate_scale, out, words)
    xps = cl_pixel_stride(x)
    if xps is None:
        raise SeaNativeError("wino_input_transform: a channels_last float32 (B,C,H,W) tensor (or channel slice), C % 4 == 0, expected")
    B, Cc, H, W = x.shape
    if gate is not None and (gate.shape != x.shape or cl_pixel_stride(gate) != Cc):
        raise SeaNativeError("wino_input_transform: gate must be a dense channels_last tensor of the input's shape")
    _wino_vector(gate_scale, Cc, "wino_input_transform")
    L = lib()
    T = L.sea_wino_tiles(B, H, W, m)
    if T <= 0:
        raise SeaNativeError("wino_input_transform: m must be 2 or 4 and the input not empty")
    A2 = (m + 2) ** 2
    if out is None:
        out = torch.empty(A2, T, Cc, dtype=torch.float32, device=x.device)
    elif (out.dtype != torch.float32 or tuple(out.shape) != (A2, T, Cc) or out.stride(2) != 1 or out.stride(1) < Cc
          or out.stride(0) != T * out.stride(1)):
        raise SeaNativeError("wino_input_transform: out must be a float32 (A*A, T, C) tensor or a channel slice of a wider one")
    vec4 = (WINO_IN_VEC4 & 1) if vec4 is None else int(bool(vec4))
    if amax is None or amax is False:
        _check(L.sea_wino_input_transform(_p(x), xps, _p(gate), _p(gate_scale), _p(out), out.stride(1), B, Cc, H, W, m, vec4,
                                          _stream()), "sea_wino_input_transform")
        return out
    if words is None:
        words = torch.zeros(T, dtype=torch.int32, device=x.device)
    elif words.dtype != torch.int32 or words.numel() != T or not words.is_contiguous():
        raise SeaNativeError("wino_input_transform: amax must be a contiguous int32 tensor of one (pre-zeroed) word per tile")
    _check(L.sea_wino_input_transform_amax(_p(x), xps, _p(gate), _p(gate_scale), _p(out), out.stride(1), B, Cc, H, W, m, vec4,
                                           _p(words), _stream()), "sea_wino_input_transform_amax")
    return out, words


def wino_output_transform(M, shape, m: int, addend=None, scale=None, bias=None, relu: bool = False, vec4: int = None,
                          out=None):
    _dev(M, addend, scale, bias, out)
    B, Cc, H, W = shape
    L = lib()
    T = L.sea_wino_tiles(B, H, W, m)
    if T <= 0 or Cc <= 0 or Cc % 4 or tuple(M.shape) != ((m + 2) ** 2, T, Cc):
        raise SeaNativeError("wino_output_transform: m = 2 or 4, C % 4 == 0 and products of shape (A*A, T, C) expected")
    if addend is not None and (tuple(addend.shape) != (B, Cc, H, W) or cl_pixel_stride(addend) != Cc):
        raise SeaNativeError("wino_output_transform: addend must be a dense channels_last (B,C,H,W) float32 tensor")
    _wino_vector(scale, Cc, "wino_output_transform")
    _wino_vector(bias, Cc, "wino_output_transform")
    if out is None:
        out = torch.empty(B, Cc, H, W, dtype=torch.float32, device=M.device, memory_format=torch.channels_last)
    elif tuple(out.shape) != (B, Cc, H, W) or cl_pixel_stride(out) != Cc:
        raise SeaNativeError("wino_output_transform: out must be a dense channels_last (B,C,H,W) float32 tensor")
    vec4 = ((WINO_IN_VEC4 >> 1) & 1) if vec4 is None else int(bool(vec4))
    _check(L.sea_wino_output_transform(_p(_f32c(M)), _p(addend), _p(scale), _p(bias), int(relu), _p(out), B, Cc, H, W, m, vec4,
                                       _stream()), "sea_wino_output_transform")
    return out


def wino_conv3x3_cl(x, U, m: int, bias=None, scale=None, relu: bool = False, gate=None, gate_scale=None,
                    addend=None, gemm_terms: int = 0):
    xs = list(x) if isinstance(x, (list, tuple)) else [x]
    _dev(*xs, U, bias, scale, gate, gate_scale, addend)
    B, _, H, W = xs[0].shape
    Cin = sum(t.shape[1] for t in xs)
    A2, Ci, Cout = U.shape
    strides = [cl_pixel_stride(t) for t in xs]
    if (any(p is None for p in strides) or any(tuple(t.shape[2:]) != (H, W) or t.shape[0] != B for t in xs) or Ci != Cin
            or A2 != (m + 2) ** 2 or Cout % 4):
        raise SeaNativeError("wino_conv3x3_cl: channels_last float32 inputs (or channel slices) and matching filters expected")
    if gate is not None and (len(xs) != 1 or gate.shape != xs[0].shape or cl_pixel_stride(gate) != Cin):
        raise SeaNativeError("wino_conv3x3_cl: gate must match the (single) input's shape and layout")
    for v, n in ((bias, Cout), (scale, Cout), (gate_scale, Cin)):
        _wino_vector(v, n, "wino_conv3x3_cl")
    if addend is not None and (tuple(addend.shape) != (B, Cout, H, W) or cl_pixel_stride(addend) != Cout):
        raise SeaNativeError("wino_conv3x3_cl: addend must be a dense channels_last (B,Cout,H,W) float32 tensor")
    T = lib().sea_wino_tiles(B, H, W, m)
    V = torch.empty(A2, T, Cin, dtype=torch.float32, device=xs[0].device)
    off = 0
    use_split = gemm_terms in (1, 2, 3, 22) and Cin % 32 == 0 and T // B >= WINO_SPLIT_MIN_TILES
    v_amax = (torch.zeros(T, dtype=torch.int32, device=xs[0].device)
              if (use_split and gemm_terms == 22 and AMAX_FROM_PRODUCERS) else None)
    for t in xs:
        wino_input_transform(t, m, gate, gate_scale, amax=v_amax, out=V[:, :, off:off + t.shape[1]])
        off += t.shape[1]
    if use_split:
        packed = U.__dict__.setdefault("_sea_packed", {})
        Up, ver = packed.get(gemm_terms, (None, None))
        if Up is None or ver != U._version:
            fresh = gemm_split_pack(U, trans=True, terms=gemm_terms)
            if Up is None or not Up.refresh_from(fresh):
                Up = fresh
                CACHE_EPOCH[0] += 1
            packed[gemm_terms] = (Up, U._version)
        Mx = gemm_split(V, Up, amax=v_amax, amax_rows=1 if v_amax is not None else 0, groups=B)
    else:
        with torch.autocast("cuda", enabled=False):
            Mx = _f32c(torch.bmm(V, U))
    del V
    return wino_output_transform(Mx, (B, Cout, H, W), m, addend, scale, bias, relu)


DWCONV_AB = int(os.environ.get("SEA_DWCONV_AB", "0"))


def dwconv7x7_nhwc(x, wt, bias=None, flip: bool = False, addend=None, ab: int = None):
    _dev(x, wt, bias, addend)
    B, H, W, Cc = x.shape
    if addend is not None and (addend.shape != x.shape or addend.dtype != torch.float32 or not addend.is_contiguous()):
        raise SeaNativeError("dwconv7x7_nhwc: addend must be a contiguous float32 tensor of the input's shape")
    y = torch.empty_like(x)
    _check(lib().sea_dwconv7x7_nhwc_add(_p(_f32c(x)), _p(_f32c(wt)), _p(bias), _p(addend), _p(y), B, Cc, H, W, int(flip),
                                        DWCONV_AB if ab is None else int(ab), _stream()), "sea_dwconv7x7_nhwc_add")
    return y


def dwconv7x7_nhwc_weight_grad(x, gy, want_bias: bool = True):
    _dev(x, gy)
    B, H, W, Cc = x.shape
    if gy.shape != x.shape or Cc % 4:
        raise SeaNativeError("dwconv7x7_nhwc_weight_grad: x and gy (B,H,W,C) of one shape, C % 4 == 0")
    L = lib()
    ws = torch.empty(int(L.sea_dwconv7x7_nhwc_wgrad_workspace(B, Cc, H)), dtype=torch.float32, device=x.device)
    gw = torch.empty((Cc, 1, 7, 7), dtype=torch.float32, device=x.device)
    gb = torch.empty(Cc, dtype=torch.float32, device=x.device) if want_bias else None
    _check(L.sea_dwconv7x7_nhwc_wgrad(_p(_f32c(x)), _p(_f32c(gy)), _p(gw), _p(gb), _p(ws), B, Cc, H, W, _stream()),
           "sea_dwconv7x7_nhwc_wgrad")
    return gw, gb


def nchw_to_nhwc(x, scale=None):
    _dev(x, scale)
    B, Cc, H, W = x.shape
    out = torch.empty(B, H, W, Cc, dtype=torch.float32, device=x.device)
    _check(lib().sea_nchw_to_nhwc(_p(_f32c(x)), _p(scale), _p(out), B, Cc, H * W, _stream()), "sea_nchw_to_nhwc")
    return out


def nhwc_to_nchw(y, scale=None, residual=None):
    _dev(y, scale, residual)
    B, H, W, Cc = y.shape
    out = torch.empty(B, Cc, H, W, dtype=torch.float32, device=y.device)
    _check(lib().sea_nhwc_to_nchw(_p(_f32c(y)), _p(scale), _p(None if residual is None else _f32c(residual)), _p(out),
                                  B, Cc, H * W, _stream()), "sea_nhwc_to_nchw")
    return out


def patch2x2(x_nhwc):
    _dev(x_nhwc)
    x_nhwc = _f32c(x_nhwc)
    B, H, W, Cc = x_nhwc.shape
    out = torch.empty(B * (H // 2) * (W // 2), 4 * Cc, dtype=torch.float32, device=x_nhwc.device)
    _check(lib().sea_patch2x2(_p(x_nhwc), _p(out), B, H, W, Cc, 0, _stream()), "sea_patch2x2")
    return out


def unpatch2x2(rows, B, H, W):
    _dev(rows)
    rows = _f32c(rows)
    Cc = rows.shape[1] // 4
    out = torch.empty(B, H, W, Cc, dtype=torch.float32, device=rows.device)
    _check(lib().sea_patch2x2(_p(rows), _p(out), B, H, W, Cc, 1, _stream()), "sea_patch2x2")
    return out


def attention_qkv(qkv, scale: float, terms=None):
    _dev(qkv)
    qkv = _f32c(qkv)
    B, T, three, H, D = qkv.shape
    if three != 3 or D != 64:
        raise SeaNativeError("attention_qkv expects a (B,T,3,H,64) tensor")
    out = torch.empty(B, T, H * D, dtype=torch.float32, device=qkv.device)
    lse = torch.empty(B, H, T, dtype=torch.float32, device=qkv.device)
    p = qkv.data_ptr()
    terms = attn_terms_fwd() if terms is None else int(terms)
    if terms == 22:
        ws = torch.empty(4 * B * H, dtype=torch.int32, device=qkv.device)
        _check(lib().sea_attention_fwd_f16(p, p + 4 * H * D, p + 8 * H * D, T * 3 * H * D, D, 3 * H * D, B, H, T, D, float(scale),
                                           _p(ws), _p(out), _p(lse), _stream()), "sea_attention_fwd_f16")
        return out, lse
    _check(lib().sea_attention_fwd_terms(p, p + 4 * H * D, p + 8 * H * D, T * 3 * H * D, D, 3 * H * D, B, H, T, D, float(scale),
                                         _p(out), _p(lse), terms, _stream()), "sea_attention_fwd_terms")
    return out, lse
# ... 42 lines not shown
    tu = np.ascontiguousarray(unions.detach().cpu().numpy(), dtype=np.float32)
    mt = np.array(mt_state, dtype=np.uint32)
    assert mt.shape == (625,)
    sel = np.zeros(N, dtype=np.int32)
    miou = C.c_double(0.0)
    rounds = C.c_int32(0)
    rc = lib().sea_worst_miou_greedy(ti.ctypes.data, tu.ctypes.data, A, N, Cc, mt.ctypes.data, n_rounds,
                                     C.addressof(miou), sel.ctypes.data, C.addressof(rounds))
    _check(rc, "sea_worst_miou_greedy")
    return miou.value, sel.tolist(), rounds.value, tuple(int(v) for v in mt)


CACHE_EPOCH = [0]


class PackedWeight:

    def __init__(self, data, N, K, terms, batch, src=None):
        self.data, self.N, self.K, self.terms, self.batch = data, N, K, terms, batch
        self.stride = data.numel() // batch
        self.src = src
        self.slices = {}

    def _slices_of(self, S):
        W, trans = self.src
        Ws = W.view(S, self.K // S, self.N) if trans else W.view(self.N, S, self.K // S).permute(1, 0, 2)
        return gemm_split_pack(Ws, trans=trans, terms=self.terms)

    def k_slices(self, S):
        if S not in self.slices:
            self.slices[S] = self._slices_of(S)
            CACHE_EPOCH[0] += 1
        return self.slices[S]

    def refresh_from(self, new) -> bool:
        if (self.data.shape != new.data.shape or (self.N, self.K, self.terms, self.batch) != (new.N, new.K, new.terms, new.batch)
                or (self.src is None) != (new.src is None)):
            return False
        self.data.copy_(new.data)
        self.src = new.src
        for S, sl in self.slices.items():
            sl.data.copy_(self._slices_of(S).data)
        return True


def gemm_split_pack(W, trans: bool = False, terms: int = 3) -> PackedWeight:
    _dev(W)
    if W.dtype != torch.float32 or W.dim() not in (2, 3) or W.stride(-1) != 1:
        raise SeaNativeError("gemm_split_pack: float32 (N,K) / (G,N,K) weights with a contiguous last dim expected")
    Wb = W if W.dim() == 3 else W.unsqueeze(0)
    G = Wb.shape[0]
    N, K = (Wb.shape[2], Wb.shape[1]) if trans else (Wb.shape[1], Wb.shape[2])
    L = lib()
    nbytes = L.sea_gemm_split_packed_bytes(N, K, terms)
    if nbytes < 0:
        raise SeaNativeError(f"gemm_split_pack: unsupported shape N={N} K={K} terms={terms} (K % 32 == 0, terms 1, 2, 3 or 22)")
    out = torch.empty(G, nbytes, dtype=torch.uint8, device=W.device)
    for g in range(G):
        _check(L.sea_gemm_split_pack(_p(Wb[g]), Wb.stride(1), int(trans), N, K, terms, _p(out[g]), _stream()),
               "sea_gemm_split_pack")
    return PackedWeight(out, N, K, terms, G, src=(W.detach(), trans) if (W.dim() == 2 and W.is_contiguous()) else None)


USE_MLP_FUSED = os.environ.get("SEA_MLP_FUSED", "1") != "0"
USE_CLASSIFIER = os.environ.get("SEA_CLASSIFIER", "1") != "0"


def classifier_ok(P: int, K: int, cls: int) -> bool:
    return bool(USE_CLASSIFIER and lib().sea_classifier_supported(int(P), int(K), int(cls)))


def classifier_forward(y_rows, w2d, bias, B: int, P: int):
    _dev(y_rows, w2d, bias)
    cls, K = w2d.shape
    if (y_rows.dtype != torch.float32 or y_rows.shape != (B * P, K) or not y_rows.is_contiguous() or y_rows.data_ptr() % 16
            or w2d.dtype != torch.float32 or not w2d.is_contiguous() or w2d.data_ptr() % 16
            or (bias is not None and (bias.dtype != torch.float32 or bias.numel() != cls or not bias.is_contiguous()))):
        raise SeaNativeError("classifier_forward: y (B P, K) / W (cls, K) must be contiguous, 16-byte aligned float32")
    out = torch.empty((B, cls, P), dtype=torch.float32, device=y_rows.device)
    _check(lib().sea_classifier_fwd(_p(y_rows), _p(w2d), _p(bias), _p(out), B, P, K, cls, _stream()), "sea_classifier_fwd")
    return out


def classifier_backward(g, w2d, gate=None, gate_scale=None):
    _dev(g, w2d, gate, gate_scale)
    cls, K = w2d.shape
    if (gate is None) != (gate_scale is None):
        raise SeaNativeError("classifier_backward: gate and gate_scale come together")
    if gate is not None and (gate.dtype != torch.float32 or gate.dim() != 2 or gate.shape[1] != K or not gate.is_contiguous()
                             or gate_scale.dtype != torch.float32 or gate_scale.numel() != K or not gate_scale.is_contiguous()
                             or g.dim() != 3 or gate.shape[0] != g.shape[0] * g.shape[2]):
        raise SeaNativeError("classifier_backward: gate must be contiguous float32 (B P, K) rows, gate_scale (K)")
    if (g.dtype != torch.float32 or g.dim() != 3 or g.shape[1] != cls or not g.is_contiguous()
            or w2d.dtype != torch.float32 or not w2d.is_contiguous() or w2d.data_ptr() % 16):
        raise SeaNativeError("classifier_backward: g (B, cls, P) / W (cls, K) must be contiguous float32")
    B, _, P = g.shape
    gy = torch.empty((B * P, K), dtype=torch.float32, device=g.device)
    _check(lib().sea_classifier_bwd(_p(g), _p(w2d), _p(gy), B, P, K, cls, _p(gate), _p(gate_scale), _stream()), "sea_classifier_bwd")
    return gy


def mlp_fused_ok(C: int, H: int) -> bool:
    return bool(USE_MLP_FUSED and lib().sea_mlp_fused_supported(int(C), int(H)))


def _mlp_rows(t, C, what):
    if t.dtype != torch.float32 or t.dim() != 2 or t.shape[1] != C or t.stride(1) != 1 or t.stride(0) % 4 or t.data_ptr() % 16:
        raise SeaNativeError(f"mlp_fused: {what} must be float32 (M, {C}) rows, 16-byte aligned, row stride % 4 == 0")


def _ln_args(ln, Cc):
    if ln is None:
        return None
    w, b, eps = ln
    if (w.dtype != torch.float32 or b.dtype != torch.float32 or w.numel() != Cc or b.numel() != Cc or not w.is_contiguous()
            or not b.is_contiguous() or w.data_ptr() % 16 or b.data_ptr() % 16):
        raise SeaNativeError("mlp_fused: LayerNorm weight / bias must be contiguous, 16-byte aligned float32 of C entries")
    return w, b, float(eps)


def mlp_fused_forward(x2, W1p: PackedWeight, b1, W2p: PackedWeight, b2, res, amax_x, amax_h, out=None, ln=None):
    _dev(x2, b1, b2, res, out, amax_x, amax_h, *(ln[:2] if ln is not None else ()))
    M, Cc = x2.shape
    H = W1p.N
    if (W1p.terms, W2p.terms, W1p.K, W2p.N, W2p.K, W1p.batch, W2p.batch) != (22, 22, Cc, Cc, H, 1, 1):
        raise SeaNativeError("mlp_fused_forward: fp16 x 2 packs of w1 (H x C) and w2 (C x H) expected")
    _mlp_rows(x2, Cc, "x")
    if res is not None:
        _mlp_rows(res, Cc, "res")
    if out is None:
        out = torch.empty(M, Cc, dtype=torch.float32, device=x2.device)
    _mlp_rows(out, Cc, "out")
    la = _ln_args(ln, Cc)
    if la is not None:
        _check(lib().sea_ln_mlp_fused_fwd(_p(x2), x2.stride(0), _p(la[0]), _p(la[1]), la[2], _p(W1p.data), _p(b1), _p(W2p.data),
                                          _p(b2), _p(res), res.stride(0) if res is not None else 0, _p(out), out.stride(0), M, Cc,
                                          H, _p(amax_x), _p(amax_h), _stream()), "sea_ln_mlp_fused_fwd")
        return out
    _check(lib().sea_mlp_fused_fwd(_p(x2), x2.stride(0), _p(W1p.data), _p(b1), _p(W2p.data), _p(b2), _p(res),
                                   res.stride(0) if res is not None else 0, _p(out), out.stride(0), M, Cc, H, _p(amax_x),
                                   _p(amax_h), _stream()), "sea_mlp_fused_fwd")
    return out


def mlp_fused_backward(g2, x2, W1p: PackedWeight, b1, W2tp: PackedWeight, W1tp: PackedWeight, amax_x, amax_mul, out=None,
                       ln=None):
    _dev(g2, x2, b1, out, amax_x, amax_mul)
    M, Cc = x2.shape
    H = W1p.N
    if ((W1p.terms, W2tp.terms, W1tp.terms) != (22, 22, 22) or (W1p.K, W2tp.N, W2tp.K, W1tp.N, W1tp.K) != (Cc, H, Cc, Cc, H)
            or amax_mul.dtype != torch.float32 or amax_mul.numel() != 1):
        raise SeaNativeError("mlp_fused_backward: fp16 x 2 packs of w1, w2^T, w1^T and one float32 amax_mul expected")
    _mlp_rows(x2, Cc, "x")
    _mlp_rows(g2, Cc, "g")
    if out is None:
        out = torch.empty(M, Cc, dtype=torch.float32, device=x2.device)
    _mlp_rows(out, Cc, "out")
    la = _ln_args(ln, Cc)
    if la is not None:
        _dev(*la[:2])
        _check(lib().sea_ln_mlp_fused_bwd(_p(g2), g2.stride(0), _p(x2), x2.stride(0), _p(la[0]), _p(la[1]), la[2], _p(W1p.data),
                                          _p(b1), _p(W2tp.data), _p(W1tp.data), _p(out), out.stride(0), M, Cc, H, _p(amax_x),
                                          _p(amax_mul), _stream()), "sea_ln_mlp_fused_bwd")
        return out
    _check(lib().sea_mlp_fused_bwd(_p(g2), g2.stride(0), _p(x2), x2.stride(0), _p(W1p.data), _p(b1), _p(W2tp.data),
                                   _p(W1tp.data), _p(out), out.stride(0), M, Cc, H, _p(amax_x), _p(amax_mul), _stream()),
           "sea_mlp_fused_bwd")
    return out


class AmaxPool:
    _pools = {}
    SIZE = 1024

    def __init__(self, device):
        self.buf = torch.zeros(self.SIZE, dtype=torch.int32, device=device)
        self.next = 0

    @classmethod
    def get(cls, device):
# ... 207 lines not shown
```

robust-segmentation_amd/semseg/models/convnext_upernet.py:

```python
from __future__ import annotations

import os

import torch
import torch.nn.functional as F
from torch import nn

CONVNEXT_SETTINGS = {
    "T": ([3, 3, 9, 3], [96, 192, 384, 768], 384, 0.4),
    "T_CVST": ([3, 3, 9, 3], [96, 192, 384, 768], 384, 0.4),
    "T_CVST_ROB": ([3, 3, 9, 3], [96, 192, 384, 768], 384, 0.4),
    "S_CVST": ([3, 3, 27, 3], [96, 192, 384, 768], 384, 0.3),
    "S_CVST_ROB": ([3, 3, 27, 3], [96, 192, 384, 768], 384, 0.3),
    "B": ([3, 3, 27, 3], [128, 256, 512, 1024], 512, 0.4),
}


def _fp32_fwd(fn):
    def forward(ctx, *args):
        if torch.is_autocast_enabled():
            args = [a.float() if (torch.is_tensor(a) and a.is_floating_point() and a.dtype != torch.float32) else a
                    for a in args]
            with torch.autocast("cuda", enabled=False):
                return fn(ctx, *args)
# ... 258 lines not shown
    name = f"{name}_t{terms}"
    key = (_tkey(w), trans)
    if cache.get(name + "_key") != key:
        with torch.no_grad():
            cache[name] = _stable(cache.get(name), N.gemm_split_pack(w.detach(), trans=trans, terms=terms))
        cache[name + "_key"] = key
    return cache[name]


def _frozen_mm(x2d, w, cache, name, trans=False, bias=None, relu=False, terms=None, amax=None, out_amax=None, groups=1,
               row_amax=False):
    K = w.shape[0] if trans else w.shape[1]
    terms = _terms() if terms is None else terms
    if _split_ok(x2d, K, terms):
        from .. import _native as N
        if terms != 22:
            amax = out_amax = None
        return N.gemm_split(x2d, _packed(w, cache, name, trans, terms), bias=bias, relu=relu, amax=amax, out_amax=out_amax,
                            groups=groups, row_amax=row_amax)
    wt = w if trans else w.t()
    y = torch.addmm(bias, x2d, wt) if bias is not None else x2d @ wt
    return torch.relu_(y) if relu else y


def _ln_bound_word(norm, cache):
    key = _tkey(norm.weight, norm.bias)
    if cache.get("ln_bound_key") != key:
        with torch.no_grad():
            bnd = norm.weight.numel() ** 0.5 * norm.weight.abs().max() + norm.bias.abs().max()
            cache.update(ln_bound_key=key, ln_bound=_stable(cache.get("ln_bound"), bnd.float().reshape(1).contiguous().view(torch.int32)))
    return cache["ln_bound"]


def _linear_bound_word(in_word, w, b, cache):
    key = (_tkey(w, b), in_word._version)
    if cache.get("lin_bound_key") != key or cache.get("lin_bound_in") is not in_word:
        with torch.no_grad():
            bnd = in_word.view(torch.float32) * w.abs().sum(1)
            if b is not None:
                bnd = bnd + b.abs()
            cache.update(lin_bound_key=key, lin_bound_in=in_word,
                         lin_bound=_stable(cache.get("lin_bound"), bnd.max().float().reshape(1).contiguous().view(torch.int32)))
    return cache["lin_bound"]


def _l1_bound(w, cache, dim, factor=1.0):
    key = (_tkey(w), dim, factor)
    if cache.get("l1_key") != key:
        with torch.no_grad():
            cache.update(l1_key=key, l1=_stable(cache.get("l1"), (w.detach().abs().sum(dim).max() * (factor * (1.0 + 1e-6))).float().reshape(1)))
    return cache["l1"]


class _FrozenLinear(torch.autograd.Function):

    @staticmethod
    @_fp32_fwd
    def forward(ctx, x, w, b, cache, amax=None, out_amax=None):
        ctx.w, ctx.cache, ctx.shape, ctx.terms = w, cache, x.shape, _terms()
        x2 = x.reshape(-1, x.shape[-1])
        return _frozen_mm(x2, w, cache, "lin_fwd", bias=b, amax=amax, out_amax=out_amax,
                          groups=x.shape[0] if x.dim() > 2 else 1).view(*x.shape[:-1], w.shape[0])

    @staticmethod
    @_fp32_bwd
    def backward(ctx, gy):
        g2 = gy.reshape(-1, gy.shape[-1])
        if not g2.is_contiguous():
            g2 = g2.contiguous()
        return (_frozen_mm(g2, ctx.w, ctx.cache, "lin_bwd", trans=True, terms=_bwd_terms(ctx.terms), row_amax=True,
                           groups=ctx.shape[0] if len(ctx.shape) > 2 else 1).view(ctx.shape), None, None, None, None, None)


def _linear_frozen(mod_cache, x, w, b, amax=None, out_amax=None):
    if (_terms() in (1, 2, 3, 22) and x.is_cuda and x.dtype == torch.float32 and not w.requires_grad
            and (b is None or not b.requires_grad) and w.shape[1] % 32 == 0 and not torch.is_autocast_enabled()
            and x.is_contiguous() and x.numel() // x.shape[-1] >= GEMM_MIN_ROWS):
        return _FrozenLinear.apply(x, w, b, mod_cache, amax, out_amax)
    return F.linear(x, w, b)


FUSE_MLP = int(os.environ.get("SEA_FUSE_MLP", "24"))
RELU_GATE_PROLOGUE = os.environ.get("SEA_RELU_GATE_PROLOGUE", "1") != "0"
REDUCE_ADD = os.environ.get("SEA_REDUCE_ADD", "1") != "0"
FUSE_PROLOGUE_MAX_NBLOCKS = int(os.environ.get("SEA_FUSE_PRO_NB", "3"))


def _mlp_fusable(x, w1, b1, w2, b2):
    return (FUSE_MLP >= 0 and _terms() in (1, 2, 3, 22) and x.is_cuda and x.dtype == torch.float32 and x.is_contiguous()
            and not torch.is_autocast_enabled() and x.numel() // x.shape[-1] >= GEMM_MIN_ROWS
            and w1.shape[1] % 32 == 0 and w2.shape[1] % 32 == 0 and w2.shape[0] == x.shape[-1]
            and not any(t is not None and t.requires_grad for t in (w1, b1, w2, b2)))


class _FrozenMlp(torch.autograd.Function):

    @staticmethod
    @_fp32_fwd
    def forward(ctx, x, w1, b1, w2, b2, res, caches, a1, a2, ln=None):
        from .. import _native as N
        terms = _terms()
        x2 = x.reshape(-1, x.shape[-1])
        ctx.ln = None
        if terms != 22:
            a1 = a2 = None
        fuse, nb = int(FUSE_MLP), (x.shape[0] if x.dim() > 2 else 1)
        r2 = None if res is None else res.reshape(-1, res.shape[-1])
        ctx.w, ctx.b1, ctx.caches, ctx.shape, ctx.terms, ctx.has_res = (w1, w2), b1, caches, x.shape, terms, res is not None
        ctx.fuse, ctx.a1 = fuse, a1
        rows_ok = lambda t: t.stride(1) == 1 and t.stride(0) % 4 == 0 and t.data_ptr() % 16 == 0
        if (terms == 22 and fuse & 16 and a1 is not None and a2 is not None and a1.numel() == 1 and a2.numel() == 1
                and b1 is not None and N.mlp_fused_ok(w2.shape[0], w1.shape[0]) and rows_ok(x2)
                and (r2 is None or rows_ok(r2))):
            y = N.mlp_fused_forward(x2, _packed(w1, caches[0], "lin_fwd", False, terms), b1,
                                    _packed(w2, caches[1], "lin_fwd", False, terms), b2, r2, a1, a2, ln=ln)
            ctx.kernel_fused, ctx.ln = True, ln
            ctx.save_for_backward(x2)
            return y.view(x.shape)
        if ln is not None:
            raise RuntimeError("_FrozenMlp: a LayerNorm was handed in but the fused kernel does not apply (see _mlp_takes_layernorm)")
        ctx.kernel_fused = False
        t = torch.empty(x2.shape[0], w1.shape[0], dtype=torch.float32, device=x.device)
        pro = bool(fuse & 16) and -(-w2.shape[0] // 128) <= FUSE_PROLOGUE_MAX_NBLOCKS and not fuse & 1
        if pro:
            N.gemm_split(x2, _packed(w1, caches[0], "lin_fwd", False, terms), bias=b1, out=t, amax=a1, groups=nb)
            h = t
        elif fuse & 1:
            h = torch.empty_like(t)
            N.gemm_split(x2, _packed(w1, caches[0], "lin_fwd", False, terms), bias=b1, out=t, gelu_out=h, amax=a1, groups=nb)
        else:
            N.gemm_split(x2, _packed(w1, caches[0], "lin_fwd", False, terms), bias=b1, out=t, amax=a1, groups=nb)
            h = F.gelu(t)
        split2 = REDUCE_ADD and N._ksplit(x2.shape[0], w2.shape[0], w2.shape[1]) > 1
        add_in = r2 is not None and r2.is_contiguous() and (split2 or (bool(fuse & 4) and not pro))
        y = N.gemm_split(t if pro else h, _packed(w2, caches[1], "lin_fwd", False, terms), bias=b2, amax=a2, groups=nb,
                         a_gelu=pro, addend=r2 if add_in else None)
        if r2 is not None and not add_in:
            y += r2
        ctx.save_for_backward(t)
        return y.view(x.shape)

    @staticmethod
    @_fp32_bwd
    def backward(ctx, g):
        from .. import _native as N
        (t,) = ctx.saved_tensors
        terms = _bwd_terms(ctx.terms)
        g2 = g.reshape(-1, g.shape[-1])
        if not g2.is_contiguous():
            g2 = g2.contiguous()
        nb = ctx.shape[0] if len(ctx.shape) > 2 else 1
        if ctx.kernel_fused:
            x2 = t
            p1f = _packed(ctx.w[0], ctx.caches[0], "lin_fwd", False, ctx.terms)
            if terms == 22 and g2.data_ptr() % 16 == 0:
                gx = N.mlp_fused_backward(g2, x2, p1f, ctx.b1, _packed(ctx.w[1], ctx.caches[1], "lin_bwd", True, terms),
                                          _packed(ctx.w[0], ctx.caches[0], "lin_bwd", True, terms), ctx.a1,
                                          _l1_bound(ctx.w[1], ctx.caches[1], dim=0, factor=1.13), ln=ctx.ln)
                return gx.view(ctx.shape), None, None, None, None, (g if ctx.has_res else None), None, None, None, None
            if ctx.ln is not None:
                xin = x2
                x2, ln_mean, ln_rstd = N.layernorm(xin, ctx.ln[0], ctx.ln[1], ctx.ln[2])
            t = N.gemm_split(x2, p1f, bias=ctx.b1, amax=ctx.a1, groups=nb)
        p2, p1 = (_packed(ctx.w[1], ctx.caches[1], "lin_bwd", True, terms), _packed(ctx.w[0], ctx.caches[0], "lin_bwd", True, terms))
        rows = {}
        if terms == 22:
# ... 295 lines not shown
            from .. import _native as N
            gp = N.unpatch2x2(rows, B, H, W)
        else:
            gp = rows.view(B, H // 2, W // 2, 2, 2, C).permute(0, 1, 3, 2, 4, 5).reshape(B, H, W, C)
        return gp.permute(0, 3, 1, 2), None, None, None, None


def _patch_conv_ok(conv, x):
    return (USE_HIP_DWCONV and isinstance(conv, nn.Conv2d) and conv.kernel_size == (2, 2) and conv.stride == (2, 2)
            and conv.padding == (0, 0) and conv.groups == 1 and x.is_cuda and x.dtype == torch.float32
            and conv.weight.dtype == torch.float32
            and x.shape[2] % 2 == 0 and x.shape[3] % 2 == 0
            and not (conv.weight.requires_grad or (conv.bias is not None and conv.bias.requires_grad)))


class ConvNeXt(nn.Module):
    def __init__(self, strr: str, in_chans: int = 3, layer_scale_init_value: float = 1.0, out_indices=(0, 1, 2, 3)):
        super().__init__()
        if strr not in CONVNEXT_SETTINGS:
            raise AssertionError(f"ConvNeXt model name should be in {list(CONVNEXT_SETTINGS)}")
        depths, dims, _, dpr = CONVNEXT_SETTINGS[strr]
        self.variant = strr
        self.downsample_layers = nn.ModuleList()
        if "CVST" in strr:
            self.downsample_layers.append(ConvStem())
        else:
            self.downsample_layers.append(nn.Sequential(
                nn.Conv2d(in_chans, dims[0], 4, stride=4), LayerNorm(dims[0], data_format="channels_first")))
        for i in range(3):
            self.downsample_layers.append(nn.Sequential(
                LayerNorm(dims[i], data_format="channels_first"), nn.Conv2d(dims[i], dims[i + 1], 2, stride=2)))
        rates = torch.linspace(0, dpr, sum(depths)).tolist()
        self.stages = nn.ModuleList()
        k = 0
        for i in range(4):
            self.stages.append(nn.Sequential(*[
                Block(dims[i], rates[k + j], layer_scale_init_value) for j in range(depths[i])]))
            k += depths[i]
        self.out_indices = tuple(out_indices)
        for i in range(4):
            self.add_module(f"norm{i}", LayerNorm(dims[i], data_format="channels_first"))
        self.apply(self._init)

    @staticmethod
    def _init(m):
        if isinstance(m, (nn.Conv2d, nn.Linear)):
            nn.init.trunc_normal_(m.weight, std=0.02)
            if m.bias is not None:
                nn.init.zeros_(m.bias)

    def forward(self, x):
        feats = []
        for i in range(4):
            ds = self.downsample_layers[i]
            if i > 0 and _patch_conv_ok(ds[1], x):
                pc = ds[1].__dict__.setdefault("_patch_cache", {})
                from .. import _native as N
                ln_ok = _terms() == 22 and N.AMAX_FROM_PRODUCERS and not (ds[0].weight.requires_grad or ds[0].bias.requires_grad)
                x = _PatchConv2x2.apply(ds[0](x), ds[1].weight, ds[1].bias, pc, _ln_bound_word(ds[0], pc) if ln_ok else None)
            else:
                x = ds(x)
            if STAGE_ENTRY_CONTIGUOUS and not x.is_contiguous():
                x = x.contiguous()
            x = self.stages[i](x)
            if i in self.out_indices:
                feats.append(getattr(self, f"norm{i}")(x))
        return tuple(feats)


WINOGRAD_TILE = int(os.environ.get("SEA_WINOGRAD", "4"))
WINOGRAD_MIN_PIXELS = 16 * 16


class _WinoConv3x3(torch.autograd.Function):

    @staticmethod
    @_fp32_fwd
    def forward(ctx, x, weight, m, cache, scale, shift, relu):
        from .. import _native as N
        key = (_tkey(weight), m)
        if cache.get("key") != key:
            cache.update(key=key, fwd=_stable(cache.get("fwd"), N.wino_filter(weight.contiguous(), m, False)))
        ctx.cache, ctx.m, ctx.weight, ctx.relu, ctx.terms = cache, m, weight, relu, _terms()
        y = N.wino_conv3x3_cl(_dense_cl(x), cache["fwd"], m, bias=shift, scale=scale, relu=relu, gemm_terms=ctx.terms)
        if relu:
            ctx.save_for_backward(y, scale)
        return y

    @staticmethod
    @_fp32_bwd
    def backward(ctx, gy):
        from .. import _native as N
        cache = ctx.cache
        if cache.get("bwd") is None or cache.get("bwd_key") != cache.get("key"):
            cache.update(bwd=_stable(cache.get("bwd"), N.wino_filter(ctx.weight.contiguous(), ctx.m, True)), bwd_key=cache.get("key"))
        gate, gscale = ctx.saved_tensors if ctx.relu else (None, None)
        g = gy if N.cl_pixel_stride(gy) is not None else gy.contiguous(memory_format=_CL)
        gx = N.wino_conv3x3_cl(g, cache["bwd"], ctx.m, gate=gate, gate_scale=gscale, gemm_terms=_bwd_terms(ctx.terms))
        return gx, None, None, None, None, None, None


def _folded_bn(bn, conv_bias, cache):
    ts = (bn.weight, bn.bias, bn.running_mean, bn.running_var, conv_bias)
    key = _tkey(*ts)
    if cache.get("bn_key") != key:
        with torch.no_grad():
            scale = torch.rsqrt(bn.running_var + bn.eps)
            if bn.weight is not None:
                scale = scale * bn.weight
            shift = -bn.running_mean * scale
            if bn.bias is not None:
                shift = shift + bn.bias
            if conv_bias is not None:
                shift = shift + scale * conv_bias
        cache.update(bn_key=key, scale=_stable(cache.get("scale"), scale.float().contiguous()),
                     shift=_stable(cache.get("shift"), shift.float().contiguous()))
    return cache["scale"], cache["shift"]


def _wino_ok(conv, x):
    return (WINOGRAD_TILE in (2, 4) and x.is_cuda and x.dtype == torch.float32 and conv.kernel_size == (3, 3)
            and conv.stride == (1, 1) and conv.padding == (1, 1) and conv.dilation == (1, 1) and conv.groups == 1
            and conv.padding_mode == "zeros" and not conv.weight.requires_grad
            and (conv.bias is None or not conv.bias.requires_grad) and conv.in_channels % 4 == 0
            and conv.out_channels % 4 == 0 and x.shape[2] * x.shape[3] >= WINOGRAD_MIN_PIXELS
            and not torch.is_autocast_enabled())


USE_GEMM_POINTWISE = True


def _pointwise_ok(mod, x):
    conv, bn = mod.conv, mod.batch_norm
    return (USE_GEMM_POINTWISE and x.is_cuda and x.dtype == torch.float32 and conv.kernel_size == (1, 1)
            and conv.stride == (1, 1) and conv.padding == (0, 0) and conv.groups == 1 and not bn.training
            and bn.track_running_stats and isinstance(mod.activation, nn.ReLU)
            and not any(p.requires_grad for p in mod.parameters()) and not torch.is_autocast_enabled()
            and x.is_contiguous(memory_format=torch.channels_last))


class _PointwiseRelu(torch.autograd.Function):

    @staticmethod
    def forward(ctx, x2, w, shift, cache, groups=1):
        y = _frozen_mm(x2, w, cache, "pw_fwd", bias=shift, relu=True, groups=groups)
        ctx.save_for_backward(y)
        ctx.w, ctx.cache, ctx.terms, ctx.groups = w, cache, _terms(), groups
        return y

    @staticmethod
    def backward(ctx, gy):
        (y,) = ctx.saved_tensors
        terms = _bwd_terms(ctx.terms)
        if (RELU_GATE_PROLOGUE and terms in (1, 2, 22) and gy.is_contiguous() and gy.dtype == torch.float32
                and _split_ok(gy, ctx.w.shape[0], terms)):
            from .. import _native as N
            return (N.gemm_split(gy, _packed(ctx.w, ctx.cache, "pw_bwd", True, terms), a_relu_gate=y, groups=ctx.groups,
                                 row_amax=True), None, None, None, None)
        g = torch.where(y > 0, gy, torch.zeros((), dtype=gy.dtype, device=gy.device))
        return (_frozen_mm(g, ctx.w, ctx.cache, "pw_bwd", trans=True, terms=terms, groups=ctx.groups, row_amax=True), None, None,
                None, None)


class ConvModule(nn.Module):

    def __init__(self, cin, cout, kernel_size, padding=0, dilation=1):
        super().__init__()
        self.conv = nn.Conv2d(cin, cout, kernel_size, padding=padding, dilation=dilation, bias=False)
        self.batch_norm = nn.BatchNorm2d(cout)
        self.activation = nn.ReLU()

    def _pointwise(self, x):
        if not hasattr(self, "_wino_cache"):
            object.__setattr__(self, "_wino_cache", {})
        cache, w = self._wino_cache, self.conv.weight
        scale, shift = _folded_bn(self.batch_norm, self.conv.bias, cache)
        key = (_tkey(w), cache["bn_key"])
        if cache.get("pw_key") != key:
            with torch.no_grad():
                cache.update(pw_key=key, pw_w=_stable(cache.get("pw_w"), (w.view(w.shape[0], -1) * scale[:, None]).contiguous()))
        B, _, H, W = x.shape
# ... 89 lines not shown
    def forward(ctx, size, *ts):
        from .. import _native as N
        B, (H, W) = ts[0].shape[0], size
        buf = torch.empty(B, sum(t.shape[1] for t in ts), H, W, dtype=torch.float32, device=ts[0].device,
                          memory_format=_CL)
        off = 0
        for t in ts:
            sl = buf[:, off:off + t.shape[1]]
            if tuple(t.shape[2:]) == (H, W):
                sl.copy_(t)
            else:
                N.upsample_bilinear_cl(_dense_cl(t), size, out=sl)
            off += t.shape[1]
        ctx.shapes = [tuple(t.shape) for t in ts]
        return buf

    @staticmethod
    @_fp32_bwd
    def backward(ctx, g):
        from .. import _native as N
        if N.cl_pixel_stride(g) != g.shape[1]:
            g = g.contiguous(memory_format=_CL)
        grads, off = [None], 0
        for i, shp in enumerate(ctx.shapes):
            sl = g[:, off:off + shp[1]]
            off += shp[1]
            if not ctx.needs_input_grad[i + 1]:
                grads.append(None)
            elif shp[2:] == tuple(g.shape[2:]):
                grads.append(sl)
            else:
                grads.append(N.upsample_bilinear_backward_cl(sl, shp[2:]))
        return tuple(grads)


def _cl_fusable(ts, size):
    from .. import _native as N
    return (USE_HIP_UPSAMPLE and USE_HIP_UPSAMPLE_NHWC and N._is_cl(ts[0])
            and all(t.is_cuda and t.dtype == torch.float32 and t.shape[1] % 4 == 0 and t.shape[2] <= size[0]
                    and t.shape[3] <= size[1] for t in ts))


def _up_add(x, res):
    size = tuple(int(v) for v in res.shape[2:])
    if _cl_fusable([res, x], size):
        return _UpAddCL.apply(x, res)
    return res + _up(x, size)


def _up_cat(ts, size):
    size = tuple(int(v) for v in size)
    if _cl_fusable(ts, size):
        return _UpCatCL.apply(size, *ts)
    return torch.cat([t if tuple(t.shape[2:]) == size else _up(t, size) for t in ts], dim=1)


USE_FUSED_FPN_BOTTLENECK = True
LOWRES_MIN_FACTOR = 3.0


def _fpn_bottleneck_forward(ctx, m, cache, weight, scale, shift, fs, first_grad_index):
    from .. import _native as N
    B, (H, W), Cout = fs[0].shape[0], fs[0].shape[2:], weight.shape[0]
    chans = [f.shape[1] for f in fs]
    offs = [sum(chans[:i]) for i in range(len(fs))]
    hi = [i for i, f in enumerate(fs) if i == 0 or H / f.shape[2] < LOWRES_MIN_FACTOR or W / f.shape[3] < LOWRES_MIN_FACTOR]
    lo = [i for i in range(len(fs)) if i not in hi]
    key = (_tkey(weight), m, tuple(hi), tuple(chans))
    if cache.get("fpn_key") != key:
        w_hi = torch.cat([weight[:, offs[i]:offs[i] + chans[i]] for i in hi], 1).contiguous()
        cache.update(fpn_key=key, fpn_fwd=_stable(cache.get("fpn_fwd"), N.wino_filter(w_hi, m, False)),
                     fpn_bwd=_stable(cache.get("fpn_bwd"), N.wino_filter(w_hi, m, True)),
                     fpn_lo=_stable(cache.get("fpn_lo"), [weight[:, offs[i]:offs[i] + chans[i]].permute(2, 3, 0, 1)
                                                          .reshape(9 * Cout, chans[i]).contiguous() for i in lo]))
    xs = [_dense_cl(fs[i]) if tuple(fs[i].shape[2:]) == (H, W) else N.upsample_bilinear_cl(_dense_cl(fs[i]), (H, W))
          for i in hi]
    extra = None
    for j, i in enumerate(lo):
        f = _dense_cl(fs[i])
        G = _frozen_mm(f.permute(0, 2, 3, 1).reshape(-1, f.shape[1]), cache["fpn_lo"][j], cache,
                       f"fpn_lo_fwd{j}", groups=B).view(B, f.shape[2], f.shape[3], 9, Cout)
        extra = N.tap_gather(G, (H, W), extra)
    ctx.terms = _terms()
    y = N.wino_conv3x3_cl(xs, cache["fpn_fwd"], m, bias=shift, scale=scale, relu=True, addend=extra,
                          gemm_terms=ctx.terms)
    ctx.cache, ctx.m, ctx.hi, ctx.lo, ctx.chans, ctx.first = cache, m, hi, lo, chans, first_grad_index
    ctx.shapes = [tuple(f.shape) for f in fs]
    return y


def _fpn_bottleneck_backward(ctx, gz, y):
    from .. import _native as N
    cache, chans, shapes = ctx.cache, ctx.chans, ctx.shapes
    B, _, H, W = y.shape
    grads = [None] * len(shapes)
    if any(ctx.needs_input_grad[ctx.first + i] for i in ctx.hi):
        gbuf = N.wino_conv3x3_cl(gz, cache["fpn_bwd"], ctx.m, gemm_terms=_bwd_terms(ctx.terms))
        off = 0
        for i in ctx.hi:
            sl = gbuf[:, off:off + chans[i]]
            off += chans[i]
            if ctx.needs_input_grad[ctx.first + i]:
                grads[i] = sl if shapes[i][2:] == (H, W) else N.upsample_bilinear_backward_cl(sl, shapes[i][2:])
    for j, i in enumerate(ctx.lo):
        if ctx.needs_input_grad[ctx.first + i]:
            h, w = shapes[i][2:]
            dG = N.tap_gather_backward(gz, (h, w))
            grads[i] = _frozen_mm(dG.view(B * h * w, -1), cache["fpn_lo"][j], cache, f"fpn_lo_bwd{j}", trans=True,
                                  terms=_bwd_terms(ctx.terms), groups=B, row_amax=True).view(B, h, w, chans[i]).permute(0, 3, 1, 2)
    return grads


class _FpnBottleneck(torch.autograd.Function):

    @staticmethod
    @_fp32_fwd
    def forward(ctx, m, cache, weight, scale, shift, *fs):
        y = _fpn_bottleneck_forward(ctx, m, cache, weight, scale, shift, fs, 5)
        ctx.save_for_backward(y, scale)
        return y

    @staticmethod
    @_fp32_bwd
    def backward(ctx, gy):
        from .. import _native as N
        y, scale = ctx.saved_tensors
        gz = N.gate_scale(_dense_cl(gy), y, scale)
        return (None, None, None, None, None, *_fpn_bottleneck_backward(ctx, gz, y))


class _FpnBottleneckClassify(torch.autograd.Function):

    @staticmethod
    @_fp32_fwd
    def forward(ctx, m, cache, weight, scale, shift, cls_w2d, cls_bias, *fs):
        from .. import _native as N
        y = _fpn_bottleneck_forward(ctx, m, cache, weight, scale, shift, fs, 7)
        B, Cout, H, W = y.shape
        ctx.save_for_backward(y, scale)
        ctx.cls_w2d = cls_w2d
        return N.classifier_forward(y.permute(0, 2, 3, 1).reshape(B * H * W, Cout), cls_w2d, cls_bias, B, H * W).view(B, -1, H, W)

    @staticmethod
    @_fp32_bwd
    def backward(ctx, g):
        from .. import _native as N
        y, scale = ctx.saved_tensors
        B, Cout, H, W = y.shape
        gz = N.classifier_backward(g.reshape(B, g.shape[1], H * W).contiguous(), ctx.cls_w2d,
                                   gate=y.permute(0, 2, 3, 1).reshape(B * H * W, Cout), gate_scale=scale)
        gz = gz.view(B, H, W, Cout).permute(0, 3, 1, 2)
        return (None, None, None, None, None, None, None, *_fpn_bottleneck_backward(ctx, gz, y))


def _fpn_fusable(mod, outs):
    bn = mod.batch_norm
    size = tuple(outs[0].shape[2:])
    return (USE_FUSED_FPN_BOTTLENECK and _wino_ok(mod.conv, outs[0]) and mod.conv.bias is None and not bn.training
            and bn.track_running_stats and isinstance(mod.activation, nn.ReLU)
            and not any(p.requires_grad for p in bn.parameters()) and _cl_fusable(outs, size)
            and mod.conv.in_channels == sum(o.shape[1] for o in outs)
            and any(size[0] / o.shape[2] >= LOWRES_MIN_FACTOR and size[1] / o.shape[3] >= LOWRES_MIN_FACTOR
                    for o in outs[1:]))


USE_HIP_ADAPTIVE_POOL = os.environ.get("SEA_HIP_POOL", "1") != "0"


class _AdaptivePoolCL(torch.autograd.Function):

    @staticmethod
    @_fp32_fwd
    def forward(ctx, x, oh, ow):
        from .. import _native as N
        ctx.hw = (x.shape[2], x.shape[3])
        return N.adaptive_avg_pool_nhwc(x, oh, ow)

    @staticmethod
    @_fp32_bwd
    def backward(ctx, g):
        from .. import _native as N
        return N.adaptive_avg_pool_nhwc_backward(g, *ctx.hw), None, None


def _adaptive_pool(pool: nn.AdaptiveAvgPool2d, x):
    from .. import _native as N
    s = pool.output_size
    oh, ow = (s, s) if isinstance(s, int) else s
    if (USE_HIP_ADAPTIVE_POOL and x.is_cuda and x.dtype == torch.float32 and oh is not None and ow is not None
            and oh <= x.shape[2] and ow <= x.shape[3] and N.cl_pixel_stride(x) == x.shape[1]):
        return _AdaptivePoolCL.apply(x, oh, ow)
    return pool(x)


class PyramidPooling(nn.Module):

    def __init__(self, scales, cin, cout):
        super().__init__()
        for i, s in enumerate(scales):
            blk = nn.Module()
            blk.add_module("0", nn.AdaptiveAvgPool2d(s))
            blk.add_module("1", ConvModule(cin, cout, 1))
            self.add_module(str(i), blk)
        self.n = len(scales)

    def pooled(self, x):
        return [getattr(getattr(self, str(i)), "1")(_adaptive_pool(getattr(getattr(self, str(i)), "0"), x)) for i in range(self.n)]

    def forward(self, x):
        return [_up(p, x.shape[2:]) for p in self.pooled(x)]


class _ClassifierGemm(torch.autograd.Function):

    @staticmethod
    @_fp32_fwd
    def forward(ctx, y, w2d, bias):
        from .. import _native as N
        B, Cin, H, W = y.shape
        ctx.w2d, ctx.shape = w2d, (B, Cin, H, W)
        ctx.own = N.classifier_ok(H * W, Cin, w2d.shape[0]) and w2d.is_contiguous() and (bias is None or bias.is_contiguous())
        if ctx.own:
            rows = y.permute(0, 2, 3, 1).reshape(B * H * W, Cin)
            return N.classifier_forward(rows, w2d, bias, B, H * W).view(B, w2d.shape[0], H, W)
        out = torch.matmul(w2d, y.permute(0, 2, 3, 1).reshape(B, H * W, Cin).transpose(1, 2))
        if bias is not None:
            out += bias.view(1, -1, 1)
        return out.view(B, w2d.shape[0], H, W)

    @staticmethod
    @_fp32_bwd
    def backward(ctx, g):
        from .. import _native as N
        B, Cin, H, W = ctx.shape
        if ctx.own:
# ... 168 lines not shown
```

Before: 566.4.

## Store ReLU gates as packed bitmasks for FPN bottleneck backward

The Winograd output transform now emits a packed 1-bit-per-channel ReLU mask alongside the activation, using wave shuffles to transpose bits into per-pixel 32-channel words. The backward consumers (gate_scale, the classifier backward and the Winograd input transform) read this bitmask instead of the full fp32 activation. This cuts the memory traffic of reading the gate tensor in backward, and the activation no longer needs to be saved, at the cost of an extra mask write plus shuffle and bit work in the forward and backward kernels. It is enabled by default for the FPN bottleneck (flag bit 1); the ConvModule path needs bit 2, which is off by default.

```diff
diff --git a/include/sea_hip.h b/include/sea_hip.h
--- a/include/sea_hip.h
+++ b/include/sea_hip.h
@@ -132,6 +132,14 @@
                                   void* stream);
 int sea_wino_output_transform(const float* M, const float* addend, const float* scale, const float* bias,
                               int relu, float* y, int B, int C, int H, int W, int m, int vec4, void* stream);
+int sea_wino_output_transform_mask(const float* M, const float* addend, const float* scale, const float* bias,
+                                   int relu, float* y, int B, int C, int H, int W, int m, int vec4, uint32_t* relu_mask,
+                                   void* stream);
+int sea_wino_input_transform_bits(const float* x, int64_t x_pixel_stride, const uint32_t* gate_bits, const float* scale,
+                                  float* V, int64_t v_tile_stride, int B, int C, int H, int W, int m, int vec4, void* stream);
+int sea_wino_input_transform_bits_amax(const float* x, int64_t x_pixel_stride, const uint32_t* gate_bits, const float* scale,
+                                       float* V, int64_t v_tile_stride, int B, int C, int H, int W, int m, int vec4,
+                                       uint32_t* amax_out, void* stream);
 
 int sea_layernorm_fwd(const float* x, const float* w, const float* b, float* y, float* mean, float* rstd,
                       int64_t rows, int C, float eps, void* stream);
@@ -168,6 +176,8 @@
 int sea_tap_gather_bwd(const float* gz, float* dG, int B, int C, int h, int w, int H, int W, void* stream);
 int sea_gate_scale(const float* g, const float* gate, const float* scale, float* out, int64_t pixels, int C,
                    void* stream);
+int sea_gate_scale_bits(const float* g, const uint32_t* gate_bits, const float* scale, float* out, int64_t pixels, int C,
+                        void* stream);
 
 int sea_nchw_to_nhwc(const float* in, const float* scale, float* out, int B, int C, int64_t HW, void* stream);
 int sea_nhwc_to_nchw(const float* in, const float* scale, const float* residual, float* out, int B, int C,
@@ -227,6 +237,8 @@
 int sea_classifier_fwd(const float* y, const float* W, const float* bias, float* out, int B, int P, int K, int cls, void* stream);
 int sea_classifier_bwd(const float* g, const float* W, float* gy, int B, int P, int K, int cls, const float* gate,
                        const float* gate_scale, void* stream);
+int sea_classifier_bwd_bits(const float* g, const float* W, float* gy, int B, int P, int K, int cls, const uint32_t* gate_bits,
+                            const float* gate_scale, void* stream);
 int sea_mlp_fused_supported(int C, int H);
 int sea_ln_mlp_fused_fwd(const float* x, int64_t ldx, const float* ln_w, const float* ln_b, float ln_eps, const void* W1p,
                          const float* b1, const void* W2p, const float* b2, const float* res, int64_t ldres, float* y,
diff --git a/robust-segmentation_amd/csrc/classifier.hip b/robust-segmentation_amd/csrc/classifier.hip
--- a/robust-segmentation_amd/csrc/classifier.hip
+++ b/robust-segmentation_amd/csrc/classifier.hip
@@ -55,7 +55,7 @@
   }
 }
 
-template <bool GATE>
+template <bool GATE, bool BITS = false>
 __global__ __launch_bounds__(256, 2) void classifier_bwd_kernel(const float* __restrict__ g, const float* __restrict__ W,
                                                                 float* __restrict__ gy, int tiles, int P, int K, int cls,
                                                                 const float* __restrict__ gate, const float* __restrict__ scale) {
@@ -82,10 +82,12 @@
       a[s] = (s < pairs && c < cls) ? gb[(int64_t)c * P] : 0.f;
     }
     float* const orow = gy + ((int64_t)t * 32 + 4 * h) * K + r;
-    const float* const grow = GATE ? gate + ((int64_t)t * 32 + 4 * h) * K + r : nullptr;
+    const float* const grow = (GATE && !BITS) ? gate + ((int64_t)t * 32 + 4 * h) * K + r : nullptr;
+    const uint32_t* const gwrow = (GATE && BITS) ? (const uint32_t*)gate + ((int64_t)t * 32 + r) * (K >> 5) : nullptr;
     for (int n0 = 0; n0 < K; n0 += 128) {
       cf32x16 acc[4];
-      float gt[GATE ? 4 : 1][GATE ? 16 : 1];
+      float gt[(GATE && !BITS) ? 4 : 1][(GATE && !BITS) ? 16 : 1];
+      uint32_t gw[4];
       float sc[4];
 #pragma unroll
       for (int nt = 0; nt < 4; ++nt) {
@@ -94,8 +96,12 @@
         if constexpr (GATE) {
           if (n0 + 32 * nt < K) {
             sc[nt] = scale[n0 + 32 * nt + r];
-#pragma unroll
-            for (int e = 0; e < 16; ++e) gt[nt][e] = grow[(int64_t)((e & 3) + 8 * (e >> 2)) * K + n0 + 32 * nt];
+            if constexpr (BITS) {
+              gw[nt] = gwrow[(n0 >> 5) + nt];
+            } else {
+#pragma unroll
+              for (int e = 0; e < 16; ++e) gt[nt][e] = grow[(int64_t)((e & 3) + 8 * (e >> 2)) * K + n0 + 32 * nt];
+            }
           }
         }
       }
@@ -114,7 +120,10 @@
 #pragma unroll
           for (int e = 0; e < 16; ++e) {
             const int64_t o = (int64_t)((e & 3) + 8 * (e >> 2)) * K + n0 + 32 * nt;
-            if constexpr (GATE)
+            if constexpr (GATE && BITS) {
+              const uint32_t wv = (uint32_t)__shfl((int)gw[nt], (e & 3) + 8 * (e >> 2) + 4 * h, 64);
+              orow[o] = ((wv >> r) & 1u) ? acc[nt][e] * sc[nt] : 0.f;
+            } else if constexpr (GATE)
               orow[o] = gt[nt][e] > 0.f ? acc[nt][e] * sc[nt] : 0.f;
             else
               orow[o] = acc[nt][e];
@@ -156,9 +165,11 @@
   SEA_RETURN_LAST();
 }
 
-extern "C" int sea_classifier_bwd(const float* g, const float* W, float* gy, int B, int P, int K, int cls, const float* gate,
-                                  const float* gate_scale, void* stream) {
-  SEA_CHECK_ARG(g && W && gy && B > 0 && sea_classifier_supported(P, K, cls) && ((gate == nullptr) == (gate_scale == nullptr)));
+static int classifier_bwd_impl(const float* g, const float* W, float* gy, int B, int P, int K, int cls, const float* gate,
+                               const uint32_t* gate_bits, const float* gate_scale, void* stream) {
+  const bool gated = gate != nullptr || gate_bits != nullptr;
+  SEA_CHECK_ARG(g && W && gy && B > 0 && sea_classifier_supported(P, K, cls) && (gated == (gate_scale != nullptr)));
+  SEA_CHECK_ARG(!(gate && gate_bits) && (((uintptr_t)gate_bits) & 3) == 0);
   SEA_CHECK_ARG((((uintptr_t)W) & 15) == 0 && (int64_t)B * P / 32 < (1ll << 30));
   const int tiles = (int)((int64_t)B * P / 32);
   const int lds = 2 * ((cls + 1) / 2) * (K + 32) * 4;
@@ -168,9 +179,13 @@
   if (!attr_set_dev[dev & 63]) {
     (void)hipFuncSetAttribute((const void*)classifier_bwd_kernel<false>, hipFuncAttributeMaxDynamicSharedMemorySize, CLS_MAX * (1024 + 32) * 4);
     (void)hipFuncSetAttribute((const void*)classifier_bwd_kernel<true>, hipFuncAttributeMaxDynamicSharedMemorySize, CLS_MAX * (1024 + 32) * 4);
+    (void)hipFuncSetAttribute((const void*)classifier_bwd_kernel<true, true>, hipFuncAttributeMaxDynamicSharedMemorySize, CLS_MAX * (1024 + 32) * 4);
     attr_set_dev[dev & 63] = true;
   }
-  if (gate)
+  if (gate_bits)
+    hipLaunchKernelGGL((classifier_bwd_kernel<true, true>), dim3(classifier_grid(tiles)), dim3(256), (size_t)lds, (hipStream_t)stream, g, W,
+                       gy, tiles, P, K, cls, (const float*)gate_bits, gate_scale);
+  else if (gate)
     hipLaunchKernelGGL(classifier_bwd_kernel<true>, dim3(classifier_grid(tiles)), dim3(256), (size_t)lds, (hipStream_t)stream, g, W, gy,
                        tiles, P, K, cls, gate, gate_scale);
   else
@@ -178,3 +193,14 @@
                        tiles, P, K, cls, gate, gate_scale);
   SEA_RETURN_LAST();
 }
+
+extern "C" int sea_classifier_bwd(const float* g, const float* W, float* gy, int B, int P, int K, int cls, const float* gate,
+                                  const float* gate_scale, void* stream) {
+  return classifier_bwd_impl(g, W, gy, B, P, K, cls, gate, nullptr, gate_scale, stream);
+}
+
+extern "C" int sea_classifier_bwd_bits(const float* g, const float* W, float* gy, int B, int P, int K, int cls,
+                                       const uint32_t* gate_bits, const float* gate_scale, void* stream) {
+  SEA_CHECK_ARG(gate_bits != nullptr);
+  return classifier_bwd_impl(g, W, gy, B, P, K, cls, nullptr, gate_bits, gate_scale, stream);
+}
diff --git a/robust-segmentation_amd/csrc/fpn_fused.hip b/robust-segmentation_amd/csrc/fpn_fused.hip
--- a/robust-segmentation_amd/csrc/fpn_fused.hip
+++ b/robust-segmentation_amd/csrc/fpn_fused.hip
@@ -306,6 +306,17 @@
   }
 }
 
+__global__ __launch_bounds__(256) void gate_scale_bits_kernel(const float4* __restrict__ g, const uint32_t* __restrict__ bits,
+                                                              const float4* __restrict__ scale, float4* __restrict__ out, int CG,
+                                                              int64_t total) {
+  for (int64_t i = (int64_t)blockIdx.x * blockDim.x + threadIdx.x; i < total; i += (int64_t)gridDim.x * blockDim.x) {
+    const float4 s = scale[i % CG], gv = g[i];
+    const uint32_t t = bits[i >> 3] >> (((uint32_t)i & 7u) * 4u);
+    out[i] = make_float4((t & 1u) ? gv.x * s.x : 0.f, (t & 2u) ? gv.y * s.y : 0.f, (t & 4u) ? gv.z * s.z : 0.f,
+                         (t & 8u) ? gv.w * s.w : 0.f);
+  }
+}
+
 }
 
 using namespace sea;
@@ -349,3 +360,13 @@
                      (const float4*)g, (const float4*)gate, (const float4*)scale, (float4*)out, C / 4, total);
   SEA_RETURN_LAST();
 }
+
+extern "C" int sea_gate_scale_bits(const float* g, const uint32_t* gate_bits, const float* scale, float* out, int64_t pixels,
+                                   int C, void* stream) {
+  SEA_CHECK_ARG(g && gate_bits && scale && out && pixels > 0 && C > 0 && (C % 32) == 0);
+  SEA_CHECK_ARG(((((uintptr_t)g) | ((uintptr_t)scale) | ((uintptr_t)out)) & 15) == 0 && (((uintptr_t)gate_bits) & 3) == 0);
+  const int64_t total = pixels * (C / 4);
+  hipLaunchKernelGGL(gate_scale_bits_kernel, dim3(grid_for(total, 256 * 2)), dim3(256), 0, (hipStream_t)stream,
+                     (const float4*)g, gate_bits, (const float4*)scale, (float4*)out, C / 4, total);
+  SEA_RETURN_LAST();
+}
diff --git a/robust-segmentation_amd/csrc/wino_kernels.hip b/robust-segmentation_amd/csrc/wino_kernels.hip
--- a/robust-segmentation_amd/csrc/wino_kernels.hip
+++ b/robust-segmentation_amd/csrc/wino_kernels.hip
@@ -64,7 +64,7 @@
   *(typename VecT<VEC>::type*)p = r;
 }
 
-template <int M, int VEC>
+template <int M, int VEC, bool BITS = false>
 __global__ __launch_bounds__(256) void wino_input_kernel(const float* __restrict__ x, const float* __restrict__ gate,
                                                          const float* __restrict__ scale, float* __restrict__ V, int C,
                                                          int H, int W, int nTh, int nTw, int64_t T, int64_t total,
@@ -84,6 +84,18 @@
     float sc[VEC];
 #pragma unroll
     for (int e = 0; e < VEC; ++e) sc[e] = scale ? scale[cg * VEC + e] : 1.f;
+    constexpr int F = 32 / VEC, NL = (A * A + F - 1) / F;
+    const int gsh = (cg * VEC) & 31;
+    uint32_t gwl[NL];
+    if constexpr (BITS) {
+      const uint32_t* const gbits = (const uint32_t*)gate + (int64_t)b * H * W * (C >> 5) + ((cg * VEC) >> 5);
+#pragma unroll
+      for (int n = 0; n < NL; ++n) {
+        const int pix = n * F + (int)(threadIdx.x & (F - 1));
+        const int yy = y0 + pix / A, xx = x0 + pix % A;
+        gwl[n] = (pix < A * A && yy >= 0 && yy < H && xx >= 0 && xx < W) ? gbits[((int64_t)yy * W + xx) * (C >> 5)] : 0u;
+      }
+    }
     float d[A][A][VEC];
 #pragma unroll
     for (int i = 0; i < A; ++i) {
@@ -93,7 +105,11 @@
         const int xx = x0 + j;
         if (yy >= 0 && yy < H && xx >= 0 && xx < W) {
           vload<VEC>(xb + ((int64_t)yy * W + xx) * xps, d[i][j]);
-          if (gate) {
+          if constexpr (BITS) {
+            const uint32_t gw = (uint32_t)__shfl((int)gwl[(i * A + j) / F], (i * A + j) % F, F) >> gsh;
+#pragma unroll
+            for (int e = 0; e < VEC; ++e) d[i][j][e] = ((gw >> e) & 1u) ? d[i][j][e] * sc[e] : 0.f;
+          } else if (gate) {
             float gt[VEC];
             vload<VEC>(gate + base + ((int64_t)yy * W + xx) * C, gt);
 #pragma unroll
@@ -148,7 +164,7 @@
   }
 }
 
-template <int M, int VEC>
+template <int M, int VEC, bool BITS = false>
 __global__ __launch_bounds__(256) void wino_input_cols_kernel(const float* __restrict__ x, const float* __restrict__ gate,
                                                               const float* __restrict__ scale, float* __restrict__ V, int C,
                                                               int H, int W, int nTh, int nTw, int64_t T, int64_t total,
@@ -168,6 +184,18 @@
     float sc[VEC];
 #pragma unroll
     for (int e = 0; e < VEC; ++e) sc[e] = scale ? scale[cg * VEC + e] : 1.f;
+    constexpr int F = 32 / VEC, NL = (A * A + F - 1) / F;
+    const int gsh = (cg * VEC) & 31;
+    uint32_t gwl[NL];
+    if constexpr (BITS) {
+      const uint32_t* const gbits = (const uint32_t*)gate + (int64_t)b * H * W * (C >> 5) + ((cg * VEC) >> 5);
+#pragma unroll
+      for (int n = 0; n < NL; ++n) {
+        const int pix = n * F + (int)(threadIdx.x & (F - 1));
+        const int yy = y0 + pix / A, xx = x0 + pix % A;
+        gwl[n] = (pix < A * A && yy >= 0 && yy < H && xx >= 0 && xx < W) ? gbits[((int64_t)yy * W + xx) * (C >> 5)] : 0u;
+      }
+    }
     float tmp[A][A][VEC];
 #pragma unroll
     for (int j = 0; j < A; ++j) {
@@ -178,7 +206,11 @@
         const int yy = y0 + i;
         if (yy >= 0 && yy < H && xx >= 0 && xx < W) {
           vload<VEC>(xb + ((int64_t)yy * W + xx) * xps, col[i]);
-          if (gate) {
+          if constexpr (BITS) {
+            const uint32_t gw = (uint32_t)__shfl((int)gwl[(i * A + j) / F], (i * A + j) % F, F) >> gsh;
+#pragma unroll
+            for (int e = 0; e < VEC; ++e) col[i][e] = ((gw >> e) & 1u) ? col[i][e] * sc[e] : 0.f;
+          } else if (gate) {
             float gt[VEC];
             vload<VEC>(gate + base + ((int64_t)yy * W + xx) * C, gt);
 #pragma unroll
@@ -230,13 +262,24 @@
   }
 }
 
-template <int M, int VEC>
-__global__ __launch_bounds__(256) void wino_output_kernel(const float* __restrict__ Mx, const float* __restrict__ addend,
+__host__ __device__ constexpr uint32_t wino_field_mask(int vec, int k) {
+  uint32_t m = 0;
+  for (int p = 0; p < 32 / vec; ++p)
+    if ((p & k) == 0) m |= ((1u << vec) - 1u) << (vec * p);
+  return m;
+}
+
+template <int M, int VEC, bool MASK = false>
+__global__ __launch_bounds__(256, (MASK && VEC == 2) ? 4 : 1) void wino_output_kernel(const float* __restrict__ Mx, const float* __restrict__ addend,
                                                           const float* __restrict__ scale,
                                                           const float* __restrict__ bias, int relu,
                                                           float* __restrict__ y, int C, int H, int W, int nTh, int nTw,
-                                                          int64_t T, int64_t total, Divs3 dv) {
+                                                          int64_t T, int64_t total, Divs3 dv,
+                                                          uint32_t* __restrict__ relu_mask) {
   constexpr int A = M + 2;
+  constexpr int F = 32 / VEC;
+  constexpr int NW = MASK ? M * M / F : 1;
+  static_assert(!MASK || (M == 4 && (VEC == 2 || VEC == 4)), "mask: F(4,3) only");
   const bool fast = total < kFastIndexLimit;
   for (int64_t idx = (int64_t)blockIdx.x * blockDim.x + threadIdx.x; idx < total;
        idx += (int64_t)gridDim.x * blockDim.x) {
@@ -265,6 +308,9 @@
       sv[e] = scale ? scale[cg * VEC + e] : 1.f;
     }
     float* yb = y + (int64_t)b * H * W * C + (int64_t)cg * VEC;
+    uint32_t pb[NW];
+#pragma unroll
+    for (int wi = 0; wi < NW; ++wi) pb[wi] = 0u;
 #pragma unroll
     for (int p = 0; p < M; ++p) {
       const int yy = ty * M + p;
@@ -287,6 +333,30 @@
           if (relu) o[e] = fmaxf(o[e], 0.f);
         }
         if (yy < H && xx < W) vstore<VEC>(yb + ((int64_t)yy * W + xx) * C, o);
+        if constexpr (MASK) {
+          uint32_t nib = 0u;
+#pragma unroll
+          for (int e = 0; e < VEC; ++e) nib |= (o[e] > 0.f ? 1u : 0u) << e;
+          pb[(p * M + q) / F] |= nib << (VEC * ((p * M + q) % F));
+        }
+      }
+    }
+    if constexpr (MASK) {
+      const int li = threadIdx.x & (F - 1);
+      const int CW = C >> 5;
+      uint32_t* const mb = relu_mask + (int64_t)b * H * W * CW + ((cg * VEC) >> 5);
+#pragma unroll
+      for (int wi = 0; wi < NW; ++wi) {
+        uint32_t w = pb[wi];
+#pragma unroll
+        for (int k = F / 2; k > 0; k >>= 1) {
+          const uint32_t mk = wino_field_mask(VEC, k);
+          const uint32_t other = (uint32_t)__shfl_xor((int)w, k, 64);
+          w = (li & k) ? ((w & ~mk) | ((other >> (VEC * k)) & mk)) : ((w & mk) | ((other & mk) << (VEC * k)));
+        }
+        const int pi = wi * F + li;
+        const int yy = ty * M + (pi >> 2), xx = tx * M + (pi & 3);
+        if (yy < H && xx < W) mb[((int64_t)yy * W + xx) * CW] = w;
       }
     }
   }
@@ -347,22 +417,7 @@
   return (int64_t)B * ((H + m - 1) / m) * ((W + m - 1) / m);
 }
 
-static int wino_input_impl(const float* x, int64_t x_pixel_stride, const float* gate, const float* scale, float* V,
-                           int64_t v_tile_stride, int B, int C, int H, int W, int m, int vec4, uint32_t* amax_out, void* stream);
-
-extern "C" int sea_wino_input_transform(const float* x, int64_t x_pixel_stride, const float* gate, const float* scale,
-                                        float* V, int64_t v_tile_stride, int B, int C, int H, int W, int m, int vec4,
-                                        void* stream) {
-  return wino_input_impl(x, x_pixel_stride, gate, scale, V, v_tile_stride, B, C, H, W, m, vec4, nullptr, stream);
-}
-
-extern "C" int sea_wino_input_transform_amax(const float* x, int64_t x_pixel_stride, const float* gate, const float* scale,
-                                             float* V, int64_t v_tile_stride, int B, int C, int H, int W, int m, int vec4,
-                                             uint32_t* amax_out, void* stream) {
-  SEA_CHECK_ARG(amax_out != nullptr);
-  return wino_input_impl(x, x_pixel_stride, gate, scale, V, v_tile_stride, B, C, H, W, m, vec4, amax_out, stream);
-}
-
+template <bool BITS>
 static int wino_input_impl(const float* x, int64_t x_pixel_stride, const float* gate, const float* scale, float* V,
                            int64_t v_tile_stride, int B, int C, int H, int W, int m, int vec4, uint32_t* amax_out, void* stream) {
   int nTh, nTw;
@@ -370,46 +425,98 @@
   SEA_CHECK_ARG(x && V && wino_dims(B, C, H, W, m, 4, &nTh, &nTw, &T));
   SEA_CHECK_ARG(x_pixel_stride >= C && (x_pixel_stride % 4) == 0);
   SEA_CHECK_ARG(v_tile_stride >= C && (v_tile_stride % 4) == 0);
-  SEA_CHECK_ARG(((((uintptr_t)x) | ((uintptr_t)V) | ((uintptr_t)gate)) & 15) == 0);
+  if (BITS)
+    SEA_CHECK_ARG(gate != nullptr && (C % 32) == 0 && ((((uintptr_t)x) | ((uintptr_t)V)) & 15) == 0 && (((uintptr_t)gate) & 3) == 0);
+  else
+    SEA_CHECK_ARG(((((uintptr_t)x) | ((uintptr_t)V) | ((uintptr_t)gate)) & 15) == 0);
   if (m == 2) {
     const int64_t total = T * (C / 4);
-    hipLaunchKernelGGL((wino_input_kernel<2, 4>), dim3(grid_for_xcd(total, 256)), dim3(256), 0, (hipStream_t)stream, x, gate,
+    hipLaunchKernelGGL((wino_input_kernel<2, 4, BITS>), dim3(grid_for_xcd(total, 256)), dim3(256), 0, (hipStream_t)stream, x, gate,
                        scale, V, C, H, W, nTh, nTw, T, total, x_pixel_stride, v_tile_stride, xcd_order_enabled() == 2, divs3(C / 4, nTw, nTh),
                        amax_out);
   } else if (vec4) {
     const int64_t total = T * (C / 4);
-    hipLaunchKernelGGL((wino_input_cols_kernel<4, 4>), dim3(grid_for_xcd(total, 256)), dim3(256), 0, (hipStream_t)stream, x, gate,
+    hipLaunchKernelGGL((wino_input_cols_kernel<4, 4, BITS>), dim3(grid_for_xcd(total, 256)), dim3(256), 0, (hipStream_t)stream, x, gate,
                        scale, V, C, H, W, nTh, nTw, T, total, x_pixel_stride, v_tile_stride, xcd_order_enabled() == 2, divs3(C / 4, nTw, nTh),
                        amax_out);
   } else {
     const int64_t total = T * (C / 2);
-    hipLaunchKernelGGL((wino_input_kernel<4, 2>), dim3(grid_for_xcd(total, 256)), dim3(256), 0, (hipStream_t)stream, x, gate,
+    hipLaunchKernelGGL((wino_input_kernel<4, 2, BITS>), dim3(grid_for_xcd(total, 256)), dim3(256), 0, (hipStream_t)stream, x, gate,
                        scale, V, C, H, W, nTh, nTw, T, total, x_pixel_stride, v_tile_stride, xcd_order_enabled() == 2, divs3(C / 2, nTw, nTh),
                        amax_out);
   }
   SEA_RETURN_LAST();
 }
 
-extern "C" int sea_wino_output_transform(const float* Mx, const float* addend, const float* scale, const float* bias,
-                                         int relu, float* y, int B, int C, int H, int W, int m, int vec4, void* stream) {
+extern "C" int sea_wino_input_transform(const float* x, int64_t x_pixel_stride, const float* gate, const float* scale,
+                                        float* V, int64_t v_tile_stride, int B, int C, int H, int W, int m, int vec4,
+                                        void* stream) {
+  return wino_input_impl<false>(x, x_pixel_stride, gate, scale, V, v_tile_stride, B, C, H, W, m, vec4, nullptr, stream);
+}
+
+extern "C" int sea_wino_input_transform_amax(const float* x, int64_t x_pixel_stride, const float* gate, const float* scale,
+                                             float* V, int64_t v_tile_stride, int B, int C, int H, int W, int m, int vec4,
+                                             uint32_t* amax_out, void* stream) {
+  SEA_CHECK_ARG(amax_out != nullptr);
+  return wino_input_impl<false>(x, x_pixel_stride, gate, scale, V, v_tile_stride, B, C, H, W, m, vec4, amax_out, stream);
+}
+
+extern "C" int sea_wino_input_transform_bits(const float* x, int64_t x_pixel_stride, const uint32_t* gate_bits,
+                                             const float* scale, float* V, int64_t v_tile_stride, int B, int C, int H, int W,
+                                             int m, int vec4, void* stream) {
+  return wino_input_impl<true>(x, x_pixel_stride, (const float*)gate_bits, scale, V, v_tile_stride, B, C, H, W, m, vec4, nullptr,
+                               stream);
+}
+
+extern "C" int sea_wino_input_transform_bits_amax(const float* x, int64_t x_pixel_stride, const uint32_t* gate_bits,
+                                                  const float* scale, float* V, int64_t v_tile_stride, int B, int C, int H,
+                                                  int W, int m, int vec4, uint32_t* amax_out, void* stream) {
+  SEA_CHECK_ARG(amax_out != nullptr);
+  return wino_input_impl<true>(x, x_pixel_stride, (const float*)gate_bits, scale, V, v_tile_stride, B, C, H, W, m, vec4, amax_out,
+                               stream);
+}
+
+static int wino_output_impl(const float* Mx, const float* addend, const float* scale, const float* bias, int relu, float* y,
+                            int B, int C, int H, int W, int m, int vec4, uint32_t* relu_mask, void* stream) {
   int nTh, nTw;
   int64_t T;
   SEA_CHECK_ARG(Mx && y && wino_dims(B, C, H, W, m, 4, &nTh, &nTw, &T));
   SEA_CHECK_ARG(((((uintptr_t)Mx) | ((uintptr_t)y) | ((uintptr_t)addend)) & 15) == 0);
+  SEA_CHECK_ARG(relu_mask == nullptr || (m == 4 && relu != 0 && (C % 32) == 0 && (((uintptr_t)relu_mask) & 3) == 0));
   if (m == 2) {
     const int64_t total = T * (C / 4);
     hipLaunchKernelGGL((wino_output_kernel<2, 4>), dim3(grid_for(total, 256)), dim3(256), 0, (hipStream_t)stream, Mx,
-                       addend, scale, bias, relu, y, C, H, W, nTh, nTw, T, total, divs3(C / 4, nTw, nTh));
+                       addend, scale, bias, relu, y, C, H, W, nTh, nTw, T, total, divs3(C / 4, nTw, nTh), relu_mask);
   } else if (vec4) {
     const int64_t total = T * (C / 4);
-    hipLaunchKernelGGL((wino_output_kernel<4, 4>), dim3(grid_for(total, 256)), dim3(256), 0, (hipStream_t)stream, Mx,
-                       addend, scale, bias, relu, y, C, H, W, nTh, nTw, T, total, divs3(C / 4, nTw, nTh));
+    if (relu_mask)
+      hipLaunchKernelGGL((wino_output_kernel<4, 4, true>), dim3(grid_for(total, 256)), dim3(256), 0, (hipStream_t)stream, Mx,
+                         addend, scale, bias, relu, y, C, H, W, nTh, nTw, T, total, divs3(C / 4, nTw, nTh), relu_mask);
+    else
+      hipLaunchKernelGGL((wino_output_kernel<4, 4>), dim3(grid_for(total, 256)), dim3(256), 0, (hipStream_t)stream, Mx,
+                         addend, scale, bias, relu, y, C, H, W, nTh, nTw, T, total, divs3(C / 4, nTw, nTh), relu_mask);
   } else {
     const int64_t total = T * (C / 2);
-    hipLaunchKernelGGL((wino_output_kernel<4, 2>), dim3(grid_for(total, 256)), dim3(256), 0, (hipStream_t)stream, Mx,
-                       addend, scale, bias, relu, y, C, H, W, nTh, nTw, T, total, divs3(C / 2, nTw, nTh));
+    if (relu_mask)
+      hipLaunchKernelGGL((wino_output_kernel<4, 2, true>), dim3(grid_for(total, 256)), dim3(256), 0, (hipStream_t)stream, Mx,
+                         addend, scale, bias, relu, y, C, H, W, nTh, nTw, T, total, divs3(C / 2, nTw, nTh), relu_mask);
+    else
+      hipLaunchKernelGGL((wino_output_kernel<4, 2>), dim3(grid_for(total, 256)), dim3(256), 0, (hipStream_t)stream, Mx,
+                         addend, scale, bias, relu, y, C, H, W, nTh, nTw, T, total, divs3(C / 2, nTw, nTh), relu_mask);
   }
   SEA_RETURN_LAST();
+}
+
+extern "C" int sea_wino_output_transform(const float* Mx, const float* addend, const float* scale, const float* bias,
+                                         int relu, float* y, int B, int C, int H, int W, int m, int vec4, void* stream) {
+  return wino_output_impl(Mx, addend, scale, bias, relu, y, B, C, H, W, m, vec4, nullptr, stream);
+}
+
+extern "C" int sea_wino_output_transform_mask(const float* Mx, const float* addend, const float* scale, const float* bias,
+                                              int relu, float* y, int B, int C, int H, int W, int m, int vec4,
+                                              uint32_t* relu_mask, void* stream) {
+  SEA_CHECK_ARG(relu_mask != nullptr);
+  return wino_output_impl(Mx, addend, scale, bias, relu, y, B, C, H, W, m, vec4, relu_mask, stream);
 }
 
 extern "C" int sea_wino_filter_transform(const float* w, float* U, int Cout, int Cin, int m, int flip, void* stream) {
diff --git a/robust-segmentation_amd/semseg/_native.py b/robust-segmentation_amd/semseg/_native.py
--- a/robust-segmentation_amd/semseg/_native.py
+++ b/robust-segmentation_amd/semseg/_native.py
@@ -71,9 +71,13 @@
     "sea_wino_input_transform": (_i, [_vp, _i64, _vp, _vp, _vp, _i64, _i, _i, _i, _i, _i, _i, _vp]),
     "sea_wino_filter_transform": (_i, [_vp, _vp, _i, _i, _i, _i, _vp]),
     "sea_wino_output_transform": (_i, [_vp, _vp, _vp, _vp, _i, _vp, _i, _i, _i, _i, _i, _i, _vp]),
+    "sea_wino_output_transform_mask": (_i, [_vp, _vp, _vp, _vp, _i, _vp, _i, _i, _i, _i, _i, _i, _vp, _vp]),
+    "sea_wino_input_transform_bits": (_i, [_vp, _i64, _vp, _vp, _vp, _i64, _i, _i, _i, _i, _i, _i, _vp]),
+    "sea_wino_input_transform_bits_amax": (_i, [_vp, _i64, _vp, _vp, _vp, _i64, _i, _i, _i, _i, _i, _i, _vp, _vp]),
     "sea_tap_gather_fwd": (_i, [_vp, _vp, _i, _i, _i, _i, _i, _i, _i, _i, _vp]),
     "sea_tap_gather_bwd": (_i, [_vp, _vp, _i, _i, _i, _i, _i, _i, _vp]),
     "sea_gate_scale": (_i, [_vp, _vp, _vp, _vp, _i64, _i, _vp]),
+    "sea_gate_scale_bits": (_i, [_vp, _vp, _vp, _vp, _i64, _i, _vp]),
     "sea_upsample_bilinear_nhwc_fwd": (_i, [_vp, _vp, _vp, _i, _i, _i, _i, _i, _i, _i64, _vp]),
     "sea_upsample_bilinear_nhwc_bwd": (_i, [_vp, _vp, _i, _i, _i, _i, _i, _i, _i64, _vp]),
     "sea_upsample_plan": (_i, [_i, _i64, _i, _i, _i, _i, _i, _i64, _sz, _sz, _i, _i, C.POINTER(C.c_int32)]),
@@ -97,6 +101,7 @@
     "sea_classifier_supported": (_i, [_i, _i, _i]),
     "sea_classifier_fwd": (_i, [_vp, _vp, _vp, _vp, _i, _i, _i, _i, _vp]),
     "sea_classifier_bwd": (_i, [_vp, _vp, _vp, _i, _i, _i, _i, _vp, _vp, _vp]),
+    "sea_classifier_bwd_bits": (_i, [_vp, _vp, _vp, _i, _i, _i, _i, _vp, _vp, _vp]),
     "sea_probe_gelu_mismatches": (_i, [_vp, _vp]),
     "sea_probe_ln_rows": (_i, [_vp, _vp, _vp, _f, _i, _i, _vp, _vp, _vp, _vp]),
     "sea_mlp_fused_stamps": (_i, [_i, _vp, _i64, _vp, _i64, _vp, _vp, _vp, _vp, _vp, _vp, _vp, _i, _i, _vp, _vp, _vp, _vp, _vp]),
@@ -991,8 +996,41 @@
     return dG
 
 
-def gate_scale(g, gate, scale):
-    _dev(g, gate, scale)
+def relu_mask_words(pixels: int, channels: int) -> int:
+    if pixels <= 0 or channels <= 0 or channels % 32:
+        raise SeaNativeError(f"a ReLU mask needs a channel count that is a multiple of 32, got {channels} ({pixels} pixels)")
+    return int(pixels) * (int(channels) // 32)
+
+
+def _check_relu_mask(mask, pixels: int, channels: int, what: str):
+    if (not isinstance(mask, torch.Tensor) or mask.dtype != torch.int32 or not mask.is_contiguous()
+            or mask.numel() != relu_mask_words(pixels, channels)):
+        raise SeaNativeError(f"{what}: the ReLU mask must be a contiguous int32 tensor of pixels * C / 32 = "
+                             f"{pixels} * {channels // 32} words")
+
+
+def pack_relu_mask(y):
+    rows = y.permute(0, 2, 3, 1).reshape(-1, y.shape[1]) if y.dim() == 4 else y
+    P, Cc = rows.shape
+    relu_mask_words(P, Cc)
+    bits = (rows > 0).view(P, Cc // 32, 32).to(torch.int64)
+    words = (bits << torch.arange(32, device=y.device, dtype=torch.int64)).sum(-1)
+    return (words - ((words >> 31) << 32)).to(torch.int32).reshape(-1)
+
+
+def gate_scale(g, gate=None, scale=None, gate_bits=None):
+    _dev(g, gate, scale, gate_bits)
+    if (gate is None) == (gate_bits is None) or scale is None:
+        raise SeaNativeError("gate_scale: exactly one of gate / gate_bits, and a scale, expected")
+    if gate_bits is not None:
+        B, Cc, H, W = g.shape
+        if cl_pixel_stride(g) != Cc or scale.numel() != Cc:
+            raise SeaNativeError("gate_scale: dense channels_last float32 tensors of one shape expected")
+        _check_relu_mask(gate_bits, B * H * W, Cc, "gate_scale")
+        out = torch.empty_like(g)
+        _check(lib().sea_gate_scale_bits(_p(g), _p(gate_bits), _p(_f32c(scale)), _p(out), B * H * W, Cc, _stream()),
+               "sea_gate_scale_bits")
+        return out
     B, Cc, H, W = g.shape
     if cl_pixel_stride(g) != Cc or cl_pixel_stride(gate) != Cc or gate.shape != g.shape or scale.numel() != Cc:
         raise SeaNativeError("gate_scale: dense channels_last float32 tensors of one shape expected")
@@ -1183,15 +1221,19 @@
         raise SeaNativeError(f"{what}: per-channel vectors must be contiguous float32 of the channel count")
 
 
-def wino_input_transform(x, m: int, gate=None, gate_scale=None, vec4: int = None, amax=None, out=None):
+def wino_input_transform(x, m: int, gate=None, gate_scale=None, vec4: int = None, amax=None, out=None, gate_bits=None):
     words = amax if isinstance(amax, torch.Tensor) else None
-    _dev(x, gate, gate_scale, out, words)
+    _dev(x, gate, gate_scale, out, words, gate_bits)
     xps = cl_pixel_stride(x)
     if xps is None:
         raise SeaNativeError("wino_input_transform: a channels_last float32 (B,C,H,W) tensor (or channel slice), C % 4 == 0, expected")
     B, Cc, H, W = x.shape
     if gate is not None and (gate.shape != x.shape or cl_pixel_stride(gate) != Cc):
         raise SeaNativeError("wino_input_transform: gate must be a dense channels_last tensor of the input's shape")
+    if gate_bits is not None:
+        if gate is not None:
+            raise SeaNativeError("wino_input_transform: gate and gate_bits are exclusive")
+        _check_relu_mask(gate_bits, B * H * W, Cc, "wino_input_transform")
     _wino_vector(gate_scale, Cc, "wino_input_transform")
     L = lib()
     T = L.sea_wino_tiles(B, H, W, m)
@@ -1204,23 +1246,32 @@
           or out.stride(0) != T * out.stride(1)):
         raise SeaNativeError("wino_input_transform: out must be a float32 (A*A, T, C) tensor or a channel slice of a wider one")
     vec4 = (WINO_IN_VEC4 & 1) if vec4 is None else int(bool(vec4))
+    bits = gate_bits is not None
     if amax is None or amax is False:
-        _check(L.sea_wino_input_transform(_p(x), xps, _p(gate), _p(gate_scale), _p(out), out.stride(1), B, Cc, H, W, m, vec4,
-                                          _stream()), "sea_wino_input_transform")
+        fn = L.sea_wino_input_transform_bits if bits else L.sea_wino_input_transform
+        _check(fn(_p(x), xps, _p(gate_bits if bits else gate), _p(gate_scale), _p(out), out.stride(1), B, Cc, H, W, m, vec4,
+                  _stream()), "sea_wino_input_transform")
         return out
     if words is None:
         words = torch.zeros(T, dtype=torch.int32, device=x.device)
     elif words.dtype != torch.int32 or words.numel() != T or not words.is_contiguous():
         raise SeaNativeError("wino_input_transform: amax must be a contiguous int32 tensor of one (pre-zeroed) word per tile")
-    _check(L.sea_wino_input_transform_amax(_p(x), xps, _p(gate), _p(gate_scale), _p(out), out.stride(1), B, Cc, H, W, m, vec4,
-                                           _p(words), _stream()), "sea_wino_input_transform_amax")
+    fn = L.sea_wino_input_transform_bits_amax if bits else L.sea_wino_input_transform_amax
+    _check(fn(_p(x), xps, _p(gate_bits if bits else gate), _p(gate_scale), _p(out), out.stride(1), B, Cc, H, W, m, vec4,
+              _p(words), _stream()), "sea_wino_input_transform_amax")
     return out, words
 
 
+def relu_mask_ok(channels: int, m: int = 4) -> bool:
+    return m == 4 and channels > 0 and channels % 32 == 0
+
+
 def wino_output_transform(M, shape, m: int, addend=None, scale=None, bias=None, relu: bool = False, vec4: int = None,
-                          out=None):
+                          out=None, relu_mask: bool = False):
     _dev(M, addend, scale, bias, out)
     B, Cc, H, W = shape
+    if relu_mask and not (relu and relu_mask_ok(Cc, m)):
+        raise SeaNativeError("wino_output_transform: relu_mask needs relu=True, m = 4 and C % 32 == 0")
     L = lib()
     T = L.sea_wino_tiles(B, H, W, m)
     if T <= 0 or Cc <= 0 or Cc % 4 or tuple(M.shape) != ((m + 2) ** 2, T, Cc):
@@ -1234,15 +1285,20 @@
     elif tuple(out.shape) != (B, Cc, H, W) or cl_pixel_stride(out) != Cc:
         raise SeaNativeError("wino_output_transform: out must be a dense channels_last (B,C,H,W) float32 tensor")
     vec4 = ((WINO_IN_VEC4 >> 1) & 1) if vec4 is None else int(bool(vec4))
+    if relu_mask:
+        mask = torch.empty(relu_mask_words(B * H * W, Cc), dtype=torch.int32, device=M.device)
+        _check(L.sea_wino_output_transform_mask(_p(_f32c(M)), _p(addend), _p(scale), _p(bias), int(relu), _p(out), B, Cc, H, W, m,
+                                                vec4, _p(mask), _stream()), "sea_wino_output_transform_mask")
+        return out, mask
     _check(L.sea_wino_output_transform(_p(_f32c(M)), _p(addend), _p(scale), _p(bias), int(relu), _p(out), B, Cc, H, W, m, vec4,
                                        _stream()), "sea_wino_output_transform")
     return out
 
 
 def wino_conv3x3_cl(x, U, m: int, bias=None, scale=None, relu: bool = False, gate=None, gate_scale=None,
-                    addend=None, gemm_terms: int = 0):
+                    addend=None, gemm_terms: int = 0, gate_bits=None, relu_mask: bool = False):
     xs = list(x) if isinstance(x, (list, tuple)) else [x]
-    _dev(*xs, U, bias, scale, gate, gate_scale, addend)
+    _dev(*xs, U, bias, scale, gate, gate_scale, addend, gate_bits)
     B, _, H, W = xs[0].shape
     Cin = sum(t.shape[1] for t in xs)
     A2, Ci, Cout = U.shape
@@ -1252,6 +1308,10 @@
         raise SeaNativeError("wino_conv3x3_cl: channels_last float32 inputs (or channel slices) and matching filters expected")
     if gate is not None and (len(xs) != 1 or gate.shape != xs[0].shape or cl_pixel_stride(gate) != Cin):
         raise SeaNativeError("wino_conv3x3_cl: gate must match the (single) input's shape and layout")
+    if gate_bits is not None and (len(xs) != 1 or gate is not None):
+        raise SeaNativeError("wino_conv3x3_cl: gate_bits goes with a single input and is exclusive with gate")
+    if relu_mask and not (relu and relu_mask_ok(Cout, m)):
+        raise SeaNativeError("wino_conv3x3_cl: relu_mask needs relu=True, m = 4 and Cout % 32 == 0")
     for v, n in ((bias, Cout), (scale, Cout), (gate_scale, Cin)):
         _wino_vector(v, n, "wino_conv3x3_cl")
     if addend is not None and (tuple(addend.shape) != (B, Cout, H, W) or cl_pixel_stride(addend) != Cout):
@@ -1263,7 +1323,7 @@
     v_amax = (torch.zeros(T, dtype=torch.int32, device=xs[0].device)
               if (use_split and gemm_terms == 22 and AMAX_FROM_PRODUCERS) else None)
     for t in xs:
-        wino_input_transform(t, m, gate, gate_scale, amax=v_amax, out=V[:, :, off:off + t.shape[1]])
+        wino_input_transform(t, m, gate, gate_scale, amax=v_amax, out=V[:, :, off:off + t.shape[1]], gate_bits=gate_bits)
         off += t.shape[1]
     if use_split:
         packed = U.__dict__.setdefault("_sea_packed", {})
@@ -1279,7 +1339,7 @@
         with torch.autocast("cuda", enabled=False):
             Mx = _f32c(torch.bmm(V, U))
     del V
-    return wino_output_transform(Mx, (B, Cout, H, W), m, addend, scale, bias, relu)
+    return wino_output_transform(Mx, (B, Cout, H, W), m, addend, scale, bias, relu, relu_mask=relu_mask)
 
 
 DWCONV_AB = int(os.environ.get("SEA_DWCONV_AB", "0"))
@@ -1488,11 +1548,13 @@
     return out
 
 
-def classifier_backward(g, w2d, gate=None, gate_scale=None):
-    _dev(g, w2d, gate, gate_scale)
+def classifier_backward(g, w2d, gate=None, gate_scale=None, gate_bits=None):
+    _dev(g, w2d, gate, gate_scale, gate_bits)
     cls, K = w2d.shape
-    if (gate is None) != (gate_scale is None):
-        raise SeaNativeError("classifier_backward: gate and gate_scale come together")
+    if gate is not None and gate_bits is not None:
+        raise SeaNativeError("classifier_backward: gate and gate_bits are exclusive")
+    if (gate is None and gate_bits is None) != (gate_scale is None):
+        raise SeaNativeError("classifier_backward: gate (or gate_bits) and gate_scale come together")
     if gate is not None and (gate.dtype != torch.float32 or gate.dim() != 2 or gate.shape[1] != K or not gate.is_contiguous()
                              or gate_scale.dtype != torch.float32 or gate_scale.numel() != K or not gate_scale.is_contiguous()
                              or g.dim() != 3 or gate.shape[0] != g.shape[0] * g.shape[2]):
@@ -1502,6 +1564,13 @@
         raise SeaNativeError("classifier_backward: g (B, cls, P) / W (cls, K) must be contiguous float32")
     B, _, P = g.shape
     gy = torch.empty((B * P, K), dtype=torch.float32, device=g.device)
+    if gate_bits is not None:
+        if gate_scale.dtype != torch.float32 or gate_scale.numel() != K or not gate_scale.is_contiguous():
+            raise SeaNativeError("classifier_backward: gate_scale must be contiguous float32 (K)")
+        _check_relu_mask(gate_bits, B * P, K, "classifier_backward")
+        _check(lib().sea_classifier_bwd_bits(_p(g), _p(w2d), _p(gy), B, P, K, cls, _p(gate_bits), _p(gate_scale), _stream()),
+               "sea_classifier_bwd_bits")
+        return gy
     _check(lib().sea_classifier_bwd(_p(g), _p(w2d), _p(gy), B, P, K, cls, _p(gate), _p(gate_scale), _stream()), "sea_classifier_bwd")
     return gy
 
diff --git a/robust-segmentation_amd/semseg/models/convnext_upernet.py b/robust-segmentation_amd/semseg/models/convnext_upernet.py
--- a/robust-segmentation_amd/semseg/models/convnext_upernet.py
+++ b/robust-segmentation_amd/semseg/models/convnext_upernet.py
@@ -364,6 +364,7 @@
 
 FUSE_MLP = int(os.environ.get("SEA_FUSE_MLP", "24"))
 RELU_GATE_PROLOGUE = os.environ.get("SEA_RELU_GATE_PROLOGUE", "1") != "0"
+RELU_GATE_BITS = int(os.environ.get("SEA_RELU_GATE_BITS", "1"))
 REDUCE_ADD = os.environ.get("SEA_REDUCE_ADD", "1") != "0"
 FUSE_PROLOGUE_MAX_NBLOCKS = int(os.environ.get("SEA_FUSE_PRO_NB", "3"))
 
@@ -825,6 +826,12 @@
         if cache.get("key") != key:
             cache.update(key=key, fwd=_stable(cache.get("fwd"), N.wino_filter(weight.contiguous(), m, False)))
         ctx.cache, ctx.m, ctx.weight, ctx.relu, ctx.terms = cache, m, weight, relu, _terms()
+        ctx.bits = bool(relu and (RELU_GATE_BITS & 2) and N.relu_mask_ok(weight.shape[0], m))
+        if ctx.bits:
+            y, mask = N.wino_conv3x3_cl(_dense_cl(x), cache["fwd"], m, bias=shift, scale=scale, relu=True, gemm_terms=ctx.terms,
+                                        relu_mask=True)
+            ctx.save_for_backward(mask, scale)
+            return y
         y = N.wino_conv3x3_cl(_dense_cl(x), cache["fwd"], m, bias=shift, scale=scale, relu=relu, gemm_terms=ctx.terms)
         if relu:
             ctx.save_for_backward(y, scale)
@@ -839,7 +846,10 @@
             cache.update(bwd=_stable(cache.get("bwd"), N.wino_filter(ctx.weight.contiguous(), ctx.m, True)), bwd_key=cache.get("key"))
         gate, gscale = ctx.saved_tensors if ctx.relu else (None, None)
         g = gy if N.cl_pixel_stride(gy) is not None else gy.contiguous(memory_format=_CL)
-        gx = N.wino_conv3x3_cl(g, cache["bwd"], ctx.m, gate=gate, gate_scale=gscale, gemm_terms=_bwd_terms(ctx.terms))
+        if ctx.bits:
+            gx = N.wino_conv3x3_cl(g, cache["bwd"], ctx.m, gate_bits=gate, gate_scale=gscale, gemm_terms=_bwd_terms(ctx.terms))
+        else:
+            gx = N.wino_conv3x3_cl(g, cache["bwd"], ctx.m, gate=gate, gate_scale=gscale, gemm_terms=_bwd_terms(ctx.terms))
         return gx, None, None, None, None, None, None
 
 
@@ -1095,17 +1105,20 @@
                        f"fpn_lo_fwd{j}", groups=B).view(B, f.shape[2], f.shape[3], 9, Cout)
         extra = N.tap_gather(G, (H, W), extra)
     ctx.terms = _terms()
+    ctx.bits = bool((RELU_GATE_BITS & 1) and N.relu_mask_ok(Cout, m))
     y = N.wino_conv3x3_cl(xs, cache["fpn_fwd"], m, bias=shift, scale=scale, relu=True, addend=extra,
-                          gemm_terms=ctx.terms)
+                          gemm_terms=ctx.terms, relu_mask=ctx.bits)
+    y, gate = y if ctx.bits else (y, y)
     ctx.cache, ctx.m, ctx.hi, ctx.lo, ctx.chans, ctx.first = cache, m, hi, lo, chans, first_grad_index
     ctx.shapes = [tuple(f.shape) for f in fs]
-    return y
-
-
-def _fpn_bottleneck_backward(ctx, gz, y):
+    ctx.yshape = tuple(y.shape)
+    return y, gate
+
+
+def _fpn_bottleneck_backward(ctx, gz):
     from .. import _native as N
     cache, chans, shapes = ctx.cache, ctx.chans, ctx.shapes
-    B, _, H, W = y.shape
+    B, _, H, W = ctx.yshape
     grads = [None] * len(shapes)
     if any(ctx.needs_input_grad[ctx.first + i] for i in ctx.hi):
         gbuf = N.wino_conv3x3_cl(gz, cache["fpn_bwd"], ctx.m, gemm_terms=_bwd_terms(ctx.terms))
@@ -1129,17 +1142,17 @@
     @staticmethod
     @_fp32_fwd
     def forward(ctx, m, cache, weight, scale, shift, *fs):
-        y = _fpn_bottleneck_forward(ctx, m, cache, weight, scale, shift, fs, 5)
-        ctx.save_for_backward(y, scale)
+        y, gate = _fpn_bottleneck_forward(ctx, m, cache, weight, scale, shift, fs, 5)
+        ctx.save_for_backward(gate, scale)
         return y
 
     @staticmethod
     @_fp32_bwd
     def backward(ctx, gy):
         from .. import _native as N
-        y, scale = ctx.saved_tensors
-        gz = N.gate_scale(_dense_cl(gy), y, scale)
-        return (None, None, None, None, None, *_fpn_bottleneck_backward(ctx, gz, y))
+        gate, scale = ctx.saved_tensors
+        gz = N.gate_scale(_dense_cl(gy), scale=scale, **({"gate_bits": gate} if ctx.bits else {"gate": gate}))
+        return (None, None, None, None, None, *_fpn_bottleneck_backward(ctx, gz))
 
 
 class _FpnBottleneckClassify(torch.autograd.Function):
@@ -1148,9 +1161,9 @@
     @_fp32_fwd
     def forward(ctx, m, cache, weight, scale, shift, cls_w2d, cls_bias, *fs):
         from .. import _native as N
-        y = _fpn_bottleneck_forward(ctx, m, cache, weight, scale, shift, fs, 7)
+        y, gate = _fpn_bottleneck_forward(ctx, m, cache, weight, scale, shift, fs, 7)
         B, Cout, H, W = y.shape
-        ctx.save_for_backward(y, scale)
+        ctx.save_for_backward(gate, scale)
         ctx.cls_w2d = cls_w2d
         return N.classifier_forward(y.permute(0, 2, 3, 1).reshape(B * H * W, Cout), cls_w2d, cls_bias, B, H * W).view(B, -1, H, W)
 
@@ -1158,12 +1171,15 @@
     @_fp32_bwd
     def backward(ctx, g):
         from .. import _native as N
-        y, scale = ctx.saved_tensors
-        B, Cout, H, W = y.shape
-        gz = N.classifier_backward(g.reshape(B, g.shape[1], H * W).contiguous(), ctx.cls_w2d,
-                                   gate=y.permute(0, 2, 3, 1).reshape(B * H * W, Cout), gate_scale=scale)
+        gate, scale = ctx.saved_tensors
+        B, Cout, H, W = ctx.yshape
+        if ctx.bits:
+            gz = N.classifier_backward(g.reshape(B, g.shape[1], H * W).contiguous(), ctx.cls_w2d, gate_bits=gate, gate_scale=scale)
+        else:
+            gz = N.classifier_backward(g.reshape(B, g.shape[1], H * W).contiguous(), ctx.cls_w2d,
+                                       gate=gate.permute(0, 2, 3, 1).reshape(B * H * W, Cout), gate_scale=scale)
         gz = gz.view(B, H, W, Cout).permute(0, 3, 1, 2)
-        return (None, None, None, None, None, None, None, *_fpn_bottleneck_backward(ctx, gz, y))
+        return (None, None, None, None, None, None, None, *_fpn_bottleneck_backward(ctx, gz))
 
 
 def _fpn_fusable(mod, outs):
```

After: 568.5 (median of 6 runs). About the same (+0.4%).
